# zhoupc/CNMF_E

Hardware: AMD Instinct MI355X
Metric: cnmfe_iters_per_sec (higher is better)
Workload: dtype f32; 1 GPU; c3: 512x512x10000 fp32 video, K=500, ring_radius=15, 1x1 patches of distribute_data.m (1 resident blocks per GPU), spatial=hals, deconv_flag=false, bg_ssub=1; lanes_per_rank=1, parallelism=patches round-robin over 1 rank(s)

## Files before the change

### cnmf_e_amd/csrc/api.hip

```cpp
#include "common.hpp"
#include <mutex>
#include <hip/hip_fp16.h>
#include <math.h>
#include <dlfcn.h>

namespace cnmfe {
thread_local char g_err[1024] = "";

template <class S> __device__ inline float to_f32(S v) { return (float)v; }
template <> __device__ inline float to_f32<__half>(__half v) { return __half2float(v); }

template <class S>
__global__ void k_convert(const S *__restrict__ src, float *__restrict__ dst, int64_t n) {
    int64_t i = (int64_t)blockIdx.x * blockDim.x + threadIdx.x;
    int64_t stride = (int64_t)gridDim.x * blockDim.x;
    for (; i < n; i += stride) dst[i] = to_f32<S>(src[i]);
}

__global__ void k_ymean(const float *__restrict__ Y, int64_t d_b, int64_t T, double *__restrict__ ym, float *__restrict__ ymf) {
    int64_t q = (int64_t)blockIdx.x * blockDim.x + threadIdx.x;
    if (q >= d_b) return;
    double s0 = 0, s1 = 0, s2 = 0, s3 = 0;
    int64_t t = 0;
    for (; t + 3 < T; t += 4) {
        s0 += Y[(t + 0) * d_b + q]; s1 += Y[(t + 1) * d_b + q];
        s2 += Y[(t + 2) * d_b + q]; s3 += Y[(t + 3) * d_b + q];
    }
    for (; t < T; ++t) s0 += Y[t * d_b + q];
    double m = ((s0 + s1) + (s2 + s3)) / (double)T;
    ym[q] = m; ymf[q] = (float)m;
}

__global__ void k_center4(const float *__restrict__ Y, const float *__restrict__ ymf, int64_t d_b, int64_t T, float4 *__restrict__ out) {
    const int64_t q = (int64_t)blockIdx.x * blockDim.x + threadIdx.x;
    if (q >= d_b) return;
    const int64_t c = blockIdx.y;
    const float m = ymf[q];
    const int64_t t = 4 * c;
    float4 v;
    v.x = Y[t * d_b + q] - m;
    v.y = t + 1 < T ? Y[(t + 1) * d_b + q] - m : 0.f;
    v.z = t + 2 < T ? Y[(t + 2) * d_b + q] - m : 0.f;
    v.w = t + 3 < T ? Y[(t + 3) * d_b + q] - m : 0.f;
    out[c * d_b + q] = v;
}

__global__ void k_scratch_warm(int *out, int n) {
    volatile int a[144];
    for (int i = 0; i < 144; ++i) a[i] = i * n;
    int s = 0;
    for (int i = 0; i < n; ++i) s += a[(i * 7 + n) % 144];
    if (out) *out = s;
}

__global__ void k_ring_init(float *__restrict__ W, int64_t d, int nr, int p, const int *__restrict__ dr, const int *__restrict__ dc,
                            int r0, int c0, int d1, int d2) {
    int64_t m = (int64_t)blockIdx.x * blockDim.x + threadIdx.x;
    if (m >= d) return;
    int r = r0 + (int)(m % nr), c = c0 + (int)(m / nr);
    int cnt = 0;
    for (int i = 0; i < p; ++i) { int rr = r + dr[i], cc = c + dc[i]; cnt += (rr >= 1 && rr <= d1 && cc >= 1 && cc <= d2); }
    float v = cnt ? 1.0f / (float)cnt : 0.0f;
    for (int i = 0; i < p; ++i) { int rr = r + dr[i], cc = c + dc[i];
        W[(int64_t)i * d + m] = (rr >= 1 && rr <= d1 && cc >= 1 && cc <= d2) ? v : 0.0f; }
}

__global__ void k_transpose_in(const float *__restrict__ src, float *__restrict__ dst, int K, int64_t T, int64_t ldc) {
    __shared__ float tile[32][33];
    int64_t t0 = (int64_t)blockIdx.x * 32; int k0 = blockIdx.y * 32;
    for (int j = threadIdx.y; j < 32; j += blockDim.y) {
        int64_t t = t0 + j; int k = k0 + threadIdx.x;
        tile[j][threadIdx.x] = (t < T && k < K) ? src[t * K + k] : 0.f;
    }
    __syncthreads();
    for (int j = threadIdx.y; j < 32; j += blockDim.y) {
        int k = k0 + j; int64_t t = t0 + threadIdx.x;
        if (k < K && t < T) dst[(int64_t)k * ldc + t] = tile[threadIdx.x][j];
    }
}
__global__ void k_transpose_out(const float *__restrict__ src, int64_t ldc, float *__restrict__ dst, int K, int64_t T) {
    __shared__ float tile[32][33];
    int64_t t0 = (int64_t)blockIdx.x * 32; int k0 = blockIdx.y * 32;
    for (int j = threadIdx.y; j < 32; j += blockDim.y) {
        int k = k0 + j; int64_t t = t0 + threadIdx.x;
        tile[j][threadIdx.x] = (k < K && t < T) ? src[(int64_t)k * ldc + t] : 0.f;
    }
    __syncthreads();
    for (int j = threadIdx.y; j < 32; j += blockDim.y) {
        int64_t t = t0 + j; int k = k0 + threadIdx.x;
        if (t < T && k < K) dst[t * K + k] = tile[threadIdx.x][j];
    }
}

__global__ void __launch_bounds__(256) k_gather_rows(const float4 *__restrict__ src, int64_t ldc4, const int *__restrict__ idx, float4 *__restrict__ dst) {
    const float4 *s = src + (int64_t)idx[blockIdx.x] * ldc4;
    float4 *d = dst + (int64_t)blockIdx.x * ldc4;
    for (int64_t c = threadIdx.x; c < ldc4; c += 256) d[c] = s[c];
}

int upload_traces(cnmfe_ctx *ctx, DevBuf &dst, const float *C, int32_t K, int64_t T, int order, int64_t *ldc_out) {
    int64_t ldc = (T + 3) & ~int64_t(3);
    *ldc_out = ldc;
    RET(dst.ensure(std::max<int64_t>(1, (int64_t)K * ldc) * sizeof(float)));
    if (K == 0) return 0;
    if (order == CNMFE_BOUND) {
        if (!ctx->bound_valid || ctx->bound_K != K || ctx->bound_T != T)
            return fail(CNMFE_ESTATE, "no bound trace matrix of %d x %lld (cnmfe_traces_bind)", K, (long long)T);
        CK(hipMemcpyAsync(dst.p, ctx->bound.p, (size_t)K * ldc * sizeof(float), hipMemcpyDeviceToDevice, ctx->st()));
        return 0;
    }
    if (!C) return fail(CNMFE_EINVAL, "null trace matrix");
    if (order == CNMFE_BOUND_ROWS) {
        if (!ctx->bound_valid || ctx->bound_T != T) return fail(CNMFE_ESTATE, "no bound trace matrix with %lld frames (cnmfe_traces_bind)", (long long)T);
        const int32_t *rows = reinterpret_cast<const int32_t *>(C);
        for (int32_t k = 0; k < K; ++k)
            if (rows[k] < 0 || rows[k] >= ctx->bound_K) return fail(CNMFE_EINVAL, "row %d of the bound trace matrix (%d rows) does not exist", rows[k], ctx->bound_K);
        DevBuf &dIdx = ctx->tmp[15];
        RET(to_dev(ctx, dIdx, rows, (size_t)K));
        LAUNCH(ctx, "gather_rows", k_gather_rows, dim3((unsigned)K), dim3(256), 0, ctx->bound.as<float4>(), ldc >> 2, dIdx.as<int>(), dst.as<float4>());
        return 0;
    }
    CK(hipMemsetAsync(dst.p, 0, (size_t)K * ldc * sizeof(float), ctx->st()));
    if (order == CNMFE_ROWMAJOR) {
        CK(hipMemcpy2DAsync(dst.p, ldc * sizeof(float), C, T * sizeof(float), T * sizeof(float), K, hipMemcpyDefault, ctx->st()));
    } else {
        RET(ctx->stage.ensure((size_t)K * T * sizeof(float)));
        CK(hipMemcpyAsync(ctx->stage.p, C, (size_t)K * T * sizeof(float), hipMemcpyHostToDevice, ctx->st()));
        dim3 g((unsigned)((T + 31) / 32), (unsigned)((K + 31) / 32)), b(32, 8);
        LAUNCH(ctx, "transpose_in", k_transpose_in, g, b, 0, ctx->stage.as<float>(), dst.as<float>(), K, T, ldc);
    }
    CK(hipStreamSynchronize(ctx->st()));
    return 0;
}

int download_traces(cnmfe_ctx *ctx, const float *dC, int64_t ldc, float *C, int32_t K, int64_t T, int order) {
    if (K == 0 || !C) return 0;
    if (order == CNMFE_BOUND || order == CNMFE_BOUND_ROWS) order = ctx->bound_order;
    if (order == CNMFE_ROWMAJOR) {
        CK(hipMemcpy2DAsync(C, T * sizeof(float), dC, ldc * sizeof(float), T * sizeof(float), K, hipMemcpyDeviceToHost, ctx->st()));
    } else {
        RET(ctx->stage.ensure((size_t)K * T * sizeof(float)));
        dim3 g((unsigned)((T + 31) / 32), (unsigned)((K + 31) / 32)), b(32, 8);
        LAUNCH(ctx, "transpose_out", k_transpose_out, g, b, 0, dC, ldc, ctx->stage.as<float>(), K, T);
        CK(hipMemcpyAsync(C, ctx->stage.p, (size_t)K * T * sizeof(float), hipMemcpyDeviceToHost, ctx->st()));
    }
    CK(hipStreamSynchronize(ctx->st()));
    return 0;
}

__global__ void __launch_bounds__(256) k_pin_copy(PinSegs s) {
    const int g = blockIdx.y;
    const uint4 *__restrict__ src = s.src[g]; uint4 *__restrict__ dst = s.dst[g];
    const unsigned n16 = s.n16[g];
    for (unsigned i = blockIdx.x * 256u + threadIdx.x; i < n16; i += gridDim.x * 256u) dst[i] = src[i];
}
static std::mutex g_pin_mu;
static std::vector<cnmfe_ctx *> g_pin_live;
void pin_register(cnmfe_ctx *ctx, bool live) {
    std::lock_guard<std::mutex> lk(g_pin_mu);
    auto it = std::find(g_pin_live.begin(), g_pin_live.end(), ctx);
    if (live && it == g_pin_live.end()) g_pin_live.push_back(ctx);
    if (!live && it != g_pin_live.end()) g_pin_live.erase(it);
}
static void flush_locked(cnmfe_ctx *ctx) {
    if (!ctx->npseg) return;
    PinSegs &pseg = ctx->pseg;
    unsigned mx = 0;
    for (int i = 0; i < ctx->npseg; ++i) mx = std::max(mx, pseg.n16[i]);
    for (int i = ctx->npseg; i < PIN_NSEG; ++i) { pseg.src[i] = nullptr; pseg.dst[i] = nullptr; pseg.n16[i] = 0; }
    const unsigned nb = std::min<unsigned>((mx + 255) / 256, 256);
    const int n = ctx->npseg; ctx->npseg = 0;
    hipLaunchKernelGGL(k_pin_copy, dim3(nb, (unsigned)n), dim3(256), 0, ctx->stream_, pseg);
}
void pin_flush_range(const void *p, size_t bytes) {
    std::lock_guard<std::mutex> lk(g_pin_mu);
    const char *lo = (const char *)p, *hi = lo + bytes;
    int cur = -1;
    for (cnmfe_ctx *c : g_pin_live) {
        bool hit = false;
        for (int i = 0; i < c->npseg && !hit; ++i) { const char *d_ = (const char *)c->pseg.dst[i]; hit = d_ >= lo && d_ < hi; }
        if (!hit) continue;
        if (cur < 0) (void)hipGetDevice(&cur);
        if (c->device != cur) (void)hipSetDevice(c->device);
        flush_locked(c);
        if (c->device != cur) (void)hipSetDevice(cur);
    }
}
void pin_flush_all() {
    std::lock_guard<std::mutex> lk(g_pin_mu);
    int cur = -1;
    for (cnmfe_ctx *c : g_pin_live) {
        if (!c->npseg) continue;
        if (cur < 0) (void)hipGetDevice(&cur);
        if (c->device != cur) (void)hipSetDevice(c->device);
        flush_locked(c);
        if (c->device != cur) (void)hipSetDevice(cur);
    }
}
int pinned_to_dev(cnmfe_ctx *ctx, void *dst, const void *src_pinned, size_t bytes) {
    if (bytes > (size_t(8) << 20)) { CK(hipMemcpyAsync(dst, src_pinned, bytes, hipMemcpyHostToDevice, ctx->st())); return 0; }
    std::lock_guard<std::mutex> lk(g_pin_mu);
    if (ctx->npseg == PIN_NSEG) flush_locked(ctx);
    const int i = ctx->npseg++;
    ctx->pseg.src[i] = (const uint4 *)src_pinned; ctx->pseg.dst[i] = (uint4 *)dst; ctx->pseg.n16[i] = (unsigned)((bytes + 15) / 16);
    return 0;
}
}
int cnmfe_ctx::copy_batch_mark() {
    hipEvent_t e;
    if (!copy_ev_pool.empty()) { e = copy_ev_pool.back(); copy_ev_pool.pop_back(); }
    else CK(hipEventCreateWithFlags(&e, hipEventDisableTiming));
    CK(hipEventRecord(e, copy_stream));
    copy_gens.push_back({++copy_gen, e});
    return 0;
}
void cnmfe_ctx::flush_copies() {
    std::lock_guard<std::mutex> lk(cnmfe::g_pin_mu);
    cnmfe::flush_locked(this);
}
namespace cnmfe {

bool bound_rows_of(const cnmfe_ctx *ctx, const float *C, int c_order, int32_t K, std::vector<int32_t> &rows) {
    rows.clear();
    if (!ctx->bound_valid || K <= 0) return false;
    if (c_order == CNMFE_BOUND) {
        if (K != ctx->bound_K) return false;
        rows.resize((size_t)K);
        for (int32_t k = 0; k < K; ++k) rows[k] = k;
        return true;
    }
    if (c_order == CNMFE_BOUND_ROWS && C) {
        const int32_t *r = reinterpret_cast<const int32_t *>(C);
        for (int32_t k = 0; k < K; ++k) if (r[k] < 0 || r[k] >= ctx->bound_K) return false;
        rows.assign(r, r + K);
        return true;
    }
    return false;
}

int ensure_ymean(cnmfe_ctx *ctx, Patch *P) {
    if (P->ymean_valid) return 0;
    if (P->frames_uploaded < P->T) return fail(CNMFE_ESTATE, "block has %lld of %lld frames uploaded", (long long)P->frames_uploaded, (long long)P->T);
    RET(P->ymean_d.ensure(P->d_b * sizeof(double)));
    RET(P->ymean_f.ensure(P->d_b * sizeof(float)));
    LAUNCH(ctx, "ymean", k_ymean, dim3((unsigned)((P->d_b + 255) / 256)), dim3(256), 0,
           P->Y.as<float>(), P->d_b, P->T, P->ymean_d.as<double>(), P->ymean_f.as<float>());
    P->Tc = (P->T + 3) / 4;
    RET(P->Yc4.ensure((size_t)P->Tc * P->d_b * sizeof(float4)));
    LAUNCH(ctx, "center4", k_center4, dim3((unsigned)((P->d_b + 255) / 256), (unsigned)P->Tc), dim3(256), 0,
           P->Y.as<float>(), P->ymean_f.as<float>(), P->d_b, P->T, P->Yc4.as<float4>());
    CK(hipStreamSynchronize(ctx->st()));
    (void)hipFree(P->Y.p); P->Y.p = nullptr; P->Y.cap = 0;
    P->ymean_valid = true;
    return 0;
}

__global__ void k_ring_pmax(const float *__restrict__ W, int64_t d, int p, int *__restrict__ pmax) {
    int64_t m = (int64_t)blockIdx.x * blockDim.x + threadIdx.x;
    int c = 0;
    if (m < d) {
        int i = 0;
        for (; i + 16 <= p; i += 16) {
            float w[16];
#pragma unroll
            for (int u = 0; u < 16; ++u) w[u] = W[(int64_t)(i + u) * d + m];
#pragma unroll
            for (int u = 0; u < 16; ++u) c += w[u] > 0.f;
        }
        for (; i < p; ++i) c += W[(int64_t)i * d + m] > 0.f;
    }
    for (int o = 32; o > 0; o >>= 1) { int v = __shfl_xor(c, o); c = v > c ? v : c; }
    if ((threadIdx.x & 63) == 0) atomicMax(pmax, c);
}
static bool first_run_of_row(const Patch *P, const float *row0) {
    std::vector<float> u;
    const int r = P->prect[0], c = P->prect[2];
    int nvalid = 0;
    for (int i = 0; i < P->p; ++i) {
        const int rr = r + P->dr[i], cc = c + P->dc[i];
        if (rr < 1 || rr > P->d1 || cc < 1 || cc > P->d2) continue;
        ++nvalid; u.push_back(row0[i]);
    }
    if (nvalid < P->d_b) u.push_back(0.f);
    std::sort(u.begin(), u.end());
    u.erase(std::unique(u.begin(), u.end()), u.end());
    return u.size() == 2;
}
int ring_stats_enqueue(cnmfe_ctx *ctx, Patch *P) {
    const size_t bytes = 64 + (size_t)P->p * sizeof(float);
    if (!P->stat_host) CK(hipHostMalloc(&P->stat_host, bytes, hipHostMallocDefault));
    if (!P->stat_ev) CK(hipEventCreateWithFlags(&P->stat_ev, hipEventDisableTiming));
    RET(P->stat_dev.ensure(64));
    CK(hipMemsetAsync(P->stat_dev.p, 0, 64, ctx->st()));
    LAUNCH(ctx, "ring_pmax", k_ring_pmax, dim3((unsigned)((P->d + 255) / 256)), dim3(256), 0, P->W.as<float>(), P->d, P->p, P->stat_dev.as<int>());
    CK(hipMemcpyAsync(P->stat_host, P->stat_dev.p, sizeof(int), hipMemcpyDeviceToHost, ctx->st()));
    CK(hipMemcpy2DAsync((char *)P->stat_host + 64, sizeof(float), P->W.p, P->d * sizeof(float), sizeof(float), P->p, hipMemcpyDeviceToHost, ctx->st()));
    CK(hipEventRecord(P->stat_ev, ctx->st()));
    P->stat_valid = true;
    return 0;
}
int ring_stats_get(cnmfe_ctx *ctx, Patch *P, int *pmax, bool *first) {
    if (!P->stat_valid) RET(ring_stats_enqueue(ctx, P));
    CK(hipEventSynchronize(P->stat_ev));
    if (pmax) *pmax = *reinterpret_cast<const int *>(P->stat_host);
    if (first) *first = first_run_of_row(P, reinterpret_cast<const float *>((const char *)P->stat_host + 64));
    return 0;
}

int ring_first_run(cnmfe_ctx *ctx, Patch *P, bool *first) { return ring_stats_get(ctx, P, nullptr, first); }
int ctx_errflag(cnmfe_ctx *ctx, int **dflag) {
    if (!ctx->errflag.p) {
        RET(ctx->errflag.ensure(sizeof(int)));
        CK(hipMemsetAsync(ctx->errflag.p, 0, sizeof(int), ctx->st()));
    }
    *dflag = ctx->errflag.as<int>();
    return 0;
}
static int errflag_raise(cnmfe_ctx *ctx, int h, bool taken = false) {
    if (!taken) CK(hipMemsetAsync(ctx->errflag.p, 0, sizeof(int), ctx->st()));
    for (auto &kv : ctx->patches) { Patch *q = kv.second; q->ysig_valid = false; q->ysig_virtual = false; q->pend = false; q->res_ac = false; q->res_kind = 0; q->pt_valid = false; }
    ctx->bgs_patch = -1;
    if (h & 8) return fail(CNMFE_EHIP, "temporal update: the device's aa = diag(A'A) disagrees with the host-side test of a column (flag %d)", h);
    if (h & 2) return fail(CNMFE_EUNSUPPORTED, "a pixel's ring touches more than 256 footprints of A_prev (flag %d)", h);
    if (h & 4) return fail(CNMFE_EUNSUPPORTED, "bg_ssub > 1: a pixel's interpolation window meets more than 64 footprints of A_prev (flag %d)", h);
    return fail(CNMFE_ESTATE, "a kernel met an inconsistent table (flag %d): the ring regression needed a block pair the covariance table does not hold", h);
}
int ctx_check_errflag(cnmfe_ctx *ctx) {
    if (!ctx->errflag.p) { CK(hipStreamSynchronize(ctx->st())); return 0; }
    int h = 0;
    CK(hipMemcpyAsync(&h, ctx->errflag.p, sizeof(int), hipMemcpyDeviceToHost, ctx->st()));
    CK(hipStreamSynchronize(ctx->st()));
    if (!h) return 0;
    return errflag_raise(ctx, h);
}
__global__ void k_flag_take(int *__restrict__ flag, int *__restrict__ out) { *out = atomicExch(flag, 0); }
__global__ void __launch_bounds__(256) k_fetch_take(const uint4 *__restrict__ src, uint4 *__restrict__ dst, unsigned n16, int *__restrict__ flag, int *__restrict__ flag_out) {
    for (unsigned i = blockIdx.x * 256u + threadIdx.x; i < n16; i += gridDim.x * 256u) dst[i] = src[i];
    if (flag && blockIdx.x == 0 && threadIdx.x == 0) *flag_out = atomicExch(flag, 0);
}

__global__ void __launch_bounds__(256) k_stitch_add(const float *__restrict__ craw, int64_t ldc, const float *__restrict__ aa, const int *__restrict__ ind,
                                                    float *__restrict__ acc, int64_t ld, int64_t T) {
    const int j = blockIdx.y;
    const float w = aa[j];
    float *row = acc + (int64_t)ind[j] * ld;
    const int64_t t = (int64_t)blockIdx.x * 256 + threadIdx.x;
    if (t < T) row[t] += w * craw[(int64_t)j * ldc + t];
    if (t == 0) row[ld - 4] += w;
}
__global__ void __launch_bounds__(256) k_stitch_finish(const float *__restrict__ acc, int64_t ld, int64_t T, int subtract_min, float *__restrict__ out, int64_t ldc) {
    const int k = blockIdx.x;
    const float *row = acc + (int64_t)k * ld;
    float w = row[ld - 4];
    if (w == 0.f) w = 1.f;
    float mn = INFINITY;
    for (int64_t t = threadIdx.x; t < T; t += 256) mn = fminf(mn, row[t] / w);
    __shared__ float red[256];
    red[threadIdx.x] = mn; __syncthreads();
    for (int o = 128; o > 0; o >>= 1) { if ((int)threadIdx.x < o) red[threadIdx.x] = fminf(red[threadIdx.x], red[threadIdx.x + o]); __syncthreads(); }
    const float sub = subtract_min ? red[0] : 0.f;
    for (int64_t t = threadIdx.x; t < ldc; t += 256) out[(int64_t)k * ldc + t] = t < T ? row[t] / w - sub : 0.f;
}

struct Rccl {
    void *h = nullptr;
    int (*CommInitAll)(void **, int, const int *) = nullptr;
    int (*AllReduce)(const void *, void *, size_t, int, int, void *, hipStream_t) = nullptr;
    int (*GroupStart)() = nullptr; int (*GroupEnd)() = nullptr; int (*CommDestroy)(void *) = nullptr;
    const char *(*GetErrorString)(int) = nullptr;
    int load() {
        if (h) return 0;
        for (const char *n : {"librccl.so.1", "librccl.so", "/opt/rocm/lib/librccl.so.1"}) { h = dlopen(n, RTLD_NOW | RTLD_GLOBAL); if (h) break; }
        if (!h) return fail(CNMFE_EUNSUPPORTED, "cnmfe_stitch_temporal over several GPUs needs RCCL (librccl.so not found: %s)", dlerror());
        CommInitAll = (decltype(CommInitAll))dlsym(h, "ncclCommInitAll"); AllReduce = (decltype(AllReduce))dlsym(h, "ncclAllReduce");
        GroupStart = (decltype(GroupStart))dlsym(h, "ncclGroupStart"); GroupEnd = (decltype(GroupEnd))dlsym(h, "ncclGroupEnd");
        CommDestroy = (decltype(CommDestroy))dlsym(h, "ncclCommDestroy"); GetErrorString = (decltype(GetErrorString))dlsym(h, "ncclGetErrorString");
        if (!CommInitAll || !AllReduce || !GroupStart || !GroupEnd || !CommDestroy) { h = nullptr; return fail(CNMFE_EUNSUPPORTED, "librccl.so lacks the ncclCommInitAll / ncclAllReduce / ncclGroup* symbols"); }
        return 0;
    }
};
static Rccl g_rccl;
static int stitch_finish_one(cnmfe_ctx *ctx, int subtract_min, float *C_raw_out, int c_order, bool async_copy = false) {
    if (!ctx->stitch_open) return fail(CNMFE_ESTATE, "cnmfe_stitch_begin has not been called");
    const int32_t K = ctx->stitch_K; const int64_t T = ctx->stitch_T, ldc = (T + 3) & ~int64_t(3);
    CK(hipSetDevice(ctx->device));
    GlobalScope gs_(ctx); if (gs_.rc) return gs_.rc;
    RET(ctx->bound.ensure((size_t)std::max<int64_t>(1, (int64_t)K * ldc) * sizeof(float)));
    if (ctx->copy_pending) { CK(hipStreamWaitEvent(ctx->st(), ctx->ev_copy_done, 0)); ctx->copy_pending = false; }
    if (K > 0) LAUNCH(ctx, "stitch_finish", k_stitch_finish, dim3((unsigned)K), dim3(256), 0, ctx->stitch.as<float>(), ctx->stitch_ld, T, subtract_min, ctx->bound.as<float>(), ldc);
    ctx->bound_K = K; ctx->bound_T = T; ctx->bound_order = (c_order == CNMFE_COLMAJOR) ? CNMFE_COLMAJOR : CNMFE_ROWMAJOR; ctx->bound_valid = K > 0;
    ++ctx->bound_gen;
    ctx->stitch_open = false;
    if (C_raw_out && async_copy && K > 0) {
        if (!ctx->copy_stream) {
            CK(hipStreamCreateWithFlags(&ctx->copy_stream, hipStreamNonBlocking));
            CK(hipEventCreateWithFlags(&ctx->ev_bound_ready, hipEventDisableTiming));
            CK(hipEventCreateWithFlags(&ctx->ev_copy_done, hipEventDisableTiming));
        }
        CK(hipEventRecord(ctx->ev_bound_ready, ctx->st()));
        CK(hipStreamWaitEvent(ctx->copy_stream, ctx->ev_bound_ready, 0));
        CK(hipMemcpy2DAsync(C_raw_out, T * sizeof(float), ctx->bound.p, ldc * sizeof(float), T * sizeof(float), K, hipMemcpyDeviceToHost, ctx->copy_stream));
        CK(hipEventRecord(ctx->ev_copy_done, ctx->copy_stream));
        ctx->copy_pending = true;
        RET(ctx->copy_batch_mark());
        return 0;
    }
    if (C_raw_out) RET(download_traces(ctx, ctx->bound.as<float>(), ldc, C_raw_out, K, T, c_order == CNMFE_COLMAJOR ? CNMFE_COLMAJOR : CNMFE_ROWMAJOR));
    return 0;
}

static void ring_offsets(int radius, int k, std::vector<int32_t> &dr, std::vector<int32_t> &dc) {
    dr.clear(); dc.clear();
    for (int c = -radius; c <= radius; ++c)
        for (int r = -radius; r <= radius; ++r) {
            int d2 = c * c + r * r;
            if (d2 >= radius * radius && d2 < (radius + 1) * (radius + 1)) { dr.push_back(r); dc.push_back(c); }
        }
    int n = (int)dr.size();
    if (k <= 0 || k > n) return;
    std::vector<int> ids(n);
    for (int i = 0; i < n; ++i) ids[i] = i;
    std::vector<double> ang(n);
    for (int i = 0; i < n; ++i) ang[i] = atan2((double)dr[i], (double)dc[i]);
    std::stable_sort(ids.begin(), ids.end(), [&](int a, int b) { return ang[a] < ang[b]; });
    std::vector<std::pair<int, int>> sel;
    for (int j = 0; j < k; ++j) {
        double x = (k == 1) ? 1.0 : 1.0 + (double)(n - 1) * j / (double)(k - 1);
        int idx = (int)floor(x + 0.5) - 1;
        sel.push_back({dc[ids[idx]], dr[ids[idx]]});
    }
    std::sort(sel.begin(), sel.end());
    sel.erase(std::unique(sel.begin(), sel.end()), sel.end());
    dr.clear(); dc.clear();
    for (auto &s : sel) { dc.push_back(s.first); dr.push_back(s.second); }
}
}

using namespace cnmfe;

cnmfe_ctx::~cnmfe_ctx() {
    if (rccl_comm && g_rccl.CommDestroy) { (void)hipSetDevice(device); g_rccl.CommDestroy(rccl_comm); rccl_comm = nullptr; }
    for (auto &kv : patches) delete kv.second;
    prof.drain();
    if (copy_stream) { (void)hipStreamSynchronize(copy_stream); (void)hipStreamDestroy(copy_stream); }
    if (ev_bound_ready) (void)hipEventDestroy(ev_bound_ready);
    if (ev_copy_done) (void)hipEventDestroy(ev_copy_done);
    for (auto &g : copy_gens) (void)hipEventDestroy(g.second);
    for (auto e : copy_ev_pool) (void)hipEventDestroy(e);
    cnmfe::pin_register(this, false);
    for (auto *j : tjobs) delete j;
    for (auto e : tickets) (void)hipEventDestroy(e);
    if (ticket_flags) (void)hipHostFree(ticket_flags);
    if (stream_) (void)hipStreamDestroy(stream_);
    for (auto *L : lanes) delete L;
    if (ev_fork) (void)hipEventDestroy(ev_fork);
}

void cnmfe_ctx::swap_lane(cnmfe_lane &L) {
    std::swap(stream_, L.stream_); std::swap(pseg, L.pseg); std::swap(npseg, L.npseg); pin.swap(L.pin); std::swap(spatial_nnz, L.spatial_nnz);
    for (int i = 0; i < 32; ++i) vp[i].swap(L.vp[i]);
    std::swap(last_ldc, L.last_ldc);
    ysig_low.swap(L.ysig_low); up_tmp.swap(L.up_tmp); bgs_r.swap(L.bgs_r); bgs_b.swap(L.bgs_b); bgs_upr.swap(L.bgs_upr); bgs_upc.swap(L.bgs_upc);
    std::swap(bgs_patch, L.bgs_patch); std::swap(bgs_d1s, L.bgs_d1s); std::swap(bgs_dF, L.bgs_dF);
    bf.swap(L.bf); dig_smax.swap(L.dig_smax); dig_rspart.swap(L.dig_rspart); dig_scale.swap(L.dig_scale); tdig.swap(L.tdig); tscale.swap(L.tscale); gk.swap(L.gk);
    win_items.swap(L.win_items); bf2.swap(L.bf2); outl_cnt.swap(L.outl_cnt); outl_sel.swap(L.outl_sel); cov.swap(L.cov); rowsum.swap(L.rowsum);
    for (int i = 0; i < 16; ++i) tmp[i].swap(L.tmp[i]);
    for (int i = 0; i < 7; ++i) inc[i].swap(L.inc[i]);
    for (int i = 0; i < 4; ++i) stg[i].swap(L.stg[i]);
    wcodes.swap(L.wcodes); solve_fill.swap(L.solve_fill); stage.swap(L.stage);
    for (int i = 0; i < 24; ++i) scr[i].swap(L.scr[i]);
    dscr.swap(L.dscr);
}
int cnmfe_ctx::activate(int lane) {
    if (lanes.empty() || lane == cur_lane) {
        if (!lanes.empty() && lane != 0 && lanes[lane]->fork_seen != fork_gen) {
            CK(hipStreamWaitEvent(stream_, ev_fork, 0)); lanes[lane]->fork_seen = fork_gen;
        }
        if (!lanes.empty() && lane != 0) lanes[lane]->dirty = true;
        return 0;
    }
    if (lane < 0 || lane >= (int)lanes.size()) return fail(CNMFE_ESTATE, "lane %d of %d", lane, (int)lanes.size());
    if (npseg) flush_copies();
    swap_lane(*lanes[cur_lane]);
    swap_lane(*lanes[lane]);
    cur_lane = lane;
    if (lane != 0) {
        if (lanes[lane]->fork_seen != fork_gen) { CK(hipStreamWaitEvent(stream_, ev_fork, 0)); lanes[lane]->fork_seen = fork_gen; }
        lanes[lane]->dirty = true;
    }
    return 0;
}
int cnmfe_ctx::join_lanes() {
    if (lanes.empty()) return 0;
    for (int l = 1; l < (int)lanes.size(); ++l) {
        if (!lanes[l]->dirty) continue;
        RET(activate(l));
        CK(hipEventRecord(lanes[l]->ev, st()));
    }
    RET(activate(0));
    for (int l = 1; l < (int)lanes.size(); ++l)
        if (lanes[l]->dirty) { CK(hipStreamWaitEvent(st(), lanes[l]->ev, 0)); lanes[l]->dirty = false; }
    return 0;
}
int cnmfe_ctx::fork_mark() {
    if (lanes.empty()) return 0;
    RET(activate(0));
    CK(hipEventRecord(ev_fork, st()));
    ++fork_gen;
    return 0;
}
static int lanes_set(cnmfe_ctx *ctx, int64_t n) {
    if (n < 1 || n > 4) return fail(CNMFE_EINVAL, "option lanes = %lld: 1 .. 4", (long long)n);
    if (!ctx->patches.empty() && (int)std::max<size_t>(1, ctx->lanes.size()) != n) return fail(CNMFE_ESTATE, "option lanes is set before the first patch is created");
    if (n == 1 || (int)ctx->lanes.size() == n) return 0;
    CK(hipSetDevice(ctx->device));
    for (int l = 0; l < n; ++l) {
        cnmfe_lane *L = new cnmfe_lane();
        ctx->lanes.push_back(L);
        CK(hipEventCreateWithFlags(&L->ev, hipEventDisableTiming));
        if (l == 0) continue;
        CK(hipStreamCreate(&L->stream_));
        hipLaunchKernelGGL(k_scratch_warm, dim3(1), dim3(64), 0, L->stream_, (int *)nullptr, 3);
        CK(hipStreamSynchronize(L->stream_));
        if (L->pin.init(size_t(64) << 20) != 0) return fail(CNMFE_EHIP, "pinned staging arena (64 MB) of lane %d could not be allocated", l);
    }
    CK(hipEventCreateWithFlags(&ctx->ev_fork, hipEventDisableTiming));
    CK(hipEventRecord(ctx->ev_fork, ctx->st()));
    return 0;
}

extern "C" {

const char *cnmfe_last_error(void) { return g_err; }
const char *cnmfe_version(void) { return "cnmfe-mi355x 0.1 (gfx950)"; }

cnmfe_ctx *cnmfe_create(int device) {
    int n = 0;
    hipError_t e = hipGetDeviceCount(&n);
    if (e != hipSuccess || n <= 0) { fail(CNMFE_EHIP, "no HIP device visible (%s)", hipGetErrorString(e)); return nullptr; }
    if (device < 0 || device >= n) { fail(CNMFE_EINVAL, "device %d out of range (0..%d)", device, n - 1); return nullptr; }
    if (hipSetDevice(device) != hipSuccess) { fail(CNMFE_EHIP, "hipSetDevice(%d) failed", device); return nullptr; }
    cnmfe_ctx *ctx = new cnmfe_ctx();
    ctx->device = device;
    if (hipStreamCreate(&ctx->stream_) != hipSuccess) { fail(CNMFE_EHIP, "hipStreamCreate failed"); delete ctx; return nullptr; }
    if (hipStreamCreateWithFlags(&ctx->copy_stream, hipStreamNonBlocking) != hipSuccess || hipEventCreateWithFlags(&ctx->ev_bound_ready, hipEventDisableTiming) != hipSuccess ||
        hipEventCreateWithFlags(&ctx->ev_copy_done, hipEventDisableTiming) != hipSuccess) { fail(CNMFE_EHIP, "copy stream / events could not be created"); delete ctx; return nullptr; }
    pin_register(ctx, true);
    if (ctx->pin.init(size_t(64) << 20) != 0) { fail(CNMFE_EHIP, "pinned staging arena (64 MB) could not be allocated"); delete ctx; return nullptr; }
    hipLaunchKernelGGL(k_scratch_warm, dim3(1), dim3(64), 0, ctx->stream_, (int *)nullptr, 3);
    hipLaunchKernelGGL(k_scratch_warm, dim3(1), dim3(64), 0, ctx->copy_stream, (int *)nullptr, 3);
    (void)hipStreamSynchronize(ctx->stream_); (void)hipStreamSynchronize(ctx->copy_stream); (void)hipGetLastError();
    (void)tu_warm_resid(); (void)tu_warm_bg(); (void)tu_warm_factor(); (void)tu_warm_deconv(); (void)tu_warm_ssub(); (void)tu_warm_vproj();
    if (const char *env = getenv("CNMFE_OPTS")) {
        std::string s(env), applied, ignored;
        size_t pos = 0;
        while (pos < s.size()) {
            size_t end = s.find(',', pos); if (end == std::string::npos) end = s.size();
            const std::string kv = s.substr(pos, end - pos); pos = end + 1;
            const size_t eq = kv.find('=');
            if (eq == std::string::npos || eq == 0) continue;
            const int rc_ = cnmfe_set_option(ctx, kv.substr(0, eq).c_str(), strtoll(kv.c_str() + eq + 1, nullptr, 10));
            (rc_ == 0 ? applied : ignored) += (rc_ == 0 ? (applied.empty() ? "" : ",") : (ignored.empty() ? "" : ",")) + kv;
        }
        static bool said = false;
        if (!said) { said = true; fprintf(stderr, "[cnmfe] CNMFE_OPTS applied to every context: %s%s%s\n", applied.empty() ? "(none)" : applied.c_str(), ignored.empty() ? "" : "; not known to this build, ignored: ", ignored.c_str()); }
    }
    return ctx;
}

void cnmfe_destroy(cnmfe_ctx *ctx) {
    if (!ctx) return;
    (void)hipSetDevice(ctx->device);
    (void)ctx->join_lanes();
    (void)hipStreamSynchronize(ctx->st());
    delete ctx;
}

int cnmfe_synchronize(cnmfe_ctx *ctx) {
    if (!ctx) return fail(CNMFE_EINVAL, "null context");
    RET(ctx->join_lanes());
    CK(hipStreamSynchronize(ctx->st()));
    if (ctx->copy_stream) CK(hipStreamSynchronize(ctx->copy_stream));
    return ctx_check_errflag(ctx);
}

int cnmfe_set_option(cnmfe_ctx *ctx, const char *name, int64_t value) {
    if (!ctx || !name) return fail(CNMFE_EINVAL, "null argument");
    static const char *known[] = {"r1_variant", "r1_delta", "r1_lazy", "r1_defer", "r1_virtual", "gram_incremental", "prealloc", "solve_packed", "sweep_dag", "win_i8_planes", "solve_staged", "solve_inv", "solve_inv_terms", "gram_i8", "win_i8", "proj_tiled", "proj_i8", "proj_i8_planes", "ssub_virtual", "temporal_early",
                                  "solve_probe", "r1_probe", "deconv_trace", "host_trace", "debug", nullptr};
    if (!strcmp(name, "lanes")) { RET(lanes_set(ctx, value)); ctx->opts[name] = value; return 0; }
    for (int i = 0; known[i]; ++i) if (!strcmp(known[i], name)) { ctx->opts[name] = value; if (!strcmp(name, "host_trace")) ctx->trace_level = (int)value; return 0; }
    return fail(CNMFE_EINVAL, "unknown option '%s'", name);
}

int cnmfe_get_option(cnmfe_ctx *ctx, const char *name, int64_t *value) {
    if (!ctx || !name || !value) return fail(CNMFE_EINVAL, "null argument");
    const struct { const char *n; int64_t v; } counters[] = {{"temporal_early_hits", ctx->early_hits}, {"temporal_early_drops", ctx->early_drops}, {"temporal_early_declined", ctx->early_declined},
                                                              {"temporal_early_entries", ctx->early_nent}, {"temporal_proj_entries", ctx->last_nent}, {"temporal_nowait", ctx->sweep_nowait},
                                                              {"merge_trace_uploads", ctx->merge_uploads},
                                                              {"bound_K", ctx->bound_valid ? (int64_t)ctx->bound_K : 0}, {"bound_T", ctx->bound_valid ? ctx->bound_T : 0}};
    for (const auto &c : counters) if (!strcmp(c.n, name)) { *value = c.v; return 0; }
    auto it = ctx->opts.find(name);
    if (it == ctx->opts.end()) return fail(CNMFE_EINVAL, "option '%s' is unknown or was never set (its default holds)", name);
    *value = it->second;
    return 0;
}

int cnmfe_patch_create(cnmfe_ctx *ctx, int patch_id, const int32_t pr[4], const int32_t br[4], int32_t d1, int32_t d2, int64_t T) {
    if (!ctx || !pr || !br) return fail(CNMFE_EINVAL, "null argument");
    if (d1 <= 0 || d2 <= 0 || T <= 0) return fail(CNMFE_EINVAL, "bad dims d1=%d d2=%d T=%lld", d1, d2, (long long)T);
    if (!(1 <= br[0] && br[0] <= pr[0] && pr[0] <= pr[1] && pr[1] <= br[1] && br[1] <= d1 &&
          1 <= br[2] && br[2] <= pr[2] && pr[2] <= pr[3] && pr[3] <= br[3] && br[3] <= d2))
        return fail(CNMFE_EINVAL, "patch [%d %d %d %d] must lie inside block [%d %d %d %d] inside the %dx%d FOV",
                    pr[0], pr[1], pr[2], pr[3], br[0], br[1], br[2], br[3], d1, d2);
    CK(hipSetDevice(ctx->device));
    if (ctx->patches.count(patch_id)) { delete ctx->patches[patch_id]; ctx->patches.erase(patch_id); }
    ctx->early.valid = false; ctx->spatial_patch = nullptr;
    Patch *P = new Patch();
    P->lane = ctx->lanes.empty() ? 0 : (ctx->patches_created++ % (int)ctx->lanes.size());
    memcpy(P->prect, pr, sizeof(P->prect)); memcpy(P->brect, br, sizeof(P->brect));
    P->d1 = d1; P->d2 = d2; P->T = T;
    P->nr = pr[1] - pr[0] + 1; P->nc = pr[3] - pr[2] + 1;
    P->nr_b = br[1] - br[0] + 1; P->nc_b = br[3] - br[2] + 1;
    P->roff = pr[0] - br[0]; P->coff = pr[2] - br[2];
    P->d = (int64_t)P->nr * P->nc; P->d_b = (int64_t)P->nr_b * P->nc_b;
    int rc = P->Y.ensure((size_t)P->d_b * T * sizeof(float));
    if (rc) { delete P; return rc; }
    if (hipMemsetAsync(P->Y.p, 0, (size_t)P->d_b * T * sizeof(float), ctx->st()) != hipSuccess) { delete P; return fail(CNMFE_EHIP, "hipMemsetAsync of the upload staging failed"); }
    P->frame_seen.assign((size_t)T, 0);
    P->Tc = (T + 3) / 4;
    ctx->patches[patch_id] = P;
    return 0;
}

int cnmfe_upload_block(cnmfe_ctx *ctx, int patch_id, const void *Y, int dtype, int memspace, int64_t t0, int64_t nt) {
    if (!ctx || !Y) return fail(CNMFE_EINVAL, "null argument");
    Patch *P = get_patch(ctx, patch_id);
    if (!P) return fail(CNMFE_ESTATE, "patch %d not created", patch_id);
    if (t0 < 0 || nt <= 0 || t0 + nt > P->T) return fail(CNMFE_EINVAL, "frames [%lld,%lld) outside [0,%lld)", (long long)t0, (long long)(t0 + nt), (long long)P->T);
    CK(hipSetDevice(ctx->device));
    size_t esz = dtype == CNMFE_F32 ? 4 : dtype == CNMFE_F64 ? 8 : dtype == CNMFE_U16 ? 2 : dtype == CNMFE_U8 ? 1 : dtype == CNMFE_F16 ? 2 : 0;
    if (!esz) return fail(CNMFE_EINVAL, "unknown dtype %d", dtype);
    if (memspace != CNMFE_HOST && memspace != CNMFE_DEVICE) return fail(CNMFE_EINVAL, "unknown memspace %d", memspace);
    if (!P->Y.p) {
        RET(P->Y.ensure((size_t)P->d_b * P->T * sizeof(float)));
        CK(hipMemsetAsync(P->Y.p, 0, (size_t)P->d_b * P->T * sizeof(float), ctx->st()));
        P->frames_uploaded = 0;
        P->frame_seen.assign((size_t)P->T, 0);
    }
    for (int64_t t = t0; t < t0 + nt; ++t)
        if (P->frame_seen[(size_t)t]) return fail(CNMFE_EINVAL, "frame %lld of patch %d was already uploaded (chunks must not overlap; re-create the patch to replace its video)", (long long)t, patch_id);
    float *dst = P->Y.as<float>() + t0 * P->d_b;
    int64_t n = nt * P->d_b;
    if (dtype == CNMFE_F32) {
        CK(hipMemcpyAsync(dst, Y, (size_t)n * 4, memspace == CNMFE_HOST ? hipMemcpyHostToDevice : hipMemcpyDeviceToDevice, ctx->st()));
    } else {
        const int64_t slab = int64_t(1) << 26;
        for (int64_t o = 0; o < n; o += slab) {
            int64_t m = std::min(slab, n - o);
            const void *src = (const char *)Y + (size_t)o * esz;
            if (memspace == CNMFE_HOST) {
                RET(ctx->stage.ensure((size_t)m * esz));
                CK(hipMemcpyAsync(ctx->stage.p, src, (size_t)m * esz, hipMemcpyHostToDevice, ctx->st()));
                src = ctx->stage.p;
            }
            dim3 g((unsigned)std::min<int64_t>((m + 255) / 256, 65535)), b(256);
            switch (dtype) {
                case CNMFE_F64: LAUNCH(ctx, "convert", k_convert<double>, g, b, 0, (const double *)src, dst + o, m); break;
                case CNMFE_U16: LAUNCH(ctx, "convert", k_convert<uint16_t>, g, b, 0, (const uint16_t *)src, dst + o, m); break;
                case CNMFE_U8:  LAUNCH(ctx, "convert", k_convert<uint8_t>, g, b, 0, (const uint8_t *)src, dst + o, m); break;
                default:        LAUNCH(ctx, "convert", k_convert<__half>, g, b, 0, (const __half *)src, dst + o, m); break;
            }
            if (memspace == CNMFE_HOST) CK(hipStreamSynchronize(ctx->st()));
        }
    }
    CK(hipStreamSynchronize(ctx->st()));
    std::fill(P->frame_seen.begin() + t0, P->frame_seen.begin() + t0 + nt, (uint8_t)1);
    P->frames_uploaded += nt;
    P->ymean_valid = false; P->ysig_valid = false; P->base_valid = false; P->base_alt_valid = false; P->drop_systems(); P->sys_alt_valid = false; P->pt_valid = false; P->dig_valid = false; P->digp_valid = false; P->yt4_valid = false;
    return 0;
}

int cnmfe_get_ymean(cnmfe_ctx *ctx, int patch_id, double *out) {
    if (!ctx || !out) return fail(CNMFE_EINVAL, "null argument");
    Patch *P = get_patch(ctx, patch_id);
    if (!P) return fail(CNMFE_ESTATE, "patch %d not created", patch_id);
    CK(hipSetDevice(ctx->device));
    RET(ensure_ymean(ctx, P));
    CK(hipMemcpyAsync(out, P->ymean_d.p, P->d_b * sizeof(double), hipMemcpyDeviceToHost, ctx->st()));
    CK(hipStreamSynchronize(ctx->st()));
    return 0;
}

int cnmfe_ring_init(cnmfe_ctx *ctx, int patch_id, int32_t radius, int32_t num_neighbors) {
    if (!ctx) return fail(CNMFE_EINVAL, "null context");
    Patch *P = get_patch(ctx, patch_id);
    if (!P) return fail(CNMFE_ESTATE, "patch %d not created", patch_id);
    if (radius < 1 || radius > 64) return fail(CNMFE_EINVAL, "ring radius %d out of range", radius);
    CK(hipSetDevice(ctx->device));
    std::vector<int32_t> ndr, ndc;
    ring_offsets(radius, num_neighbors, ndr, ndc);
    const int32_t np_ = (int32_t)ndr.size();
    if (np_ < 1) return fail(CNMFE_EINVAL, "ring of radius %d has no neighbours", radius);
    if (np_ > PMAX_RING) return fail(CNMFE_EUNSUPPORTED, "ring with %d neighbours exceeds the supported %d", np_, PMAX_RING);
    if (radius > 24) return fail(CNMFE_EUNSUPPORTED, "ring radius %d: the block-pair covariance table of the ring regression covers radii <= 24", radius);
    int h = radius;
    if ((P->prect[0] - P->brect[0] < std::min(h, P->prect[0] - 1)) || (P->brect[1] - P->prect[1] < std::min(h, P->d1 - P->prect[1])) ||
        (P->prect[2] - P->brect[2] < std::min(h, P->prect[2] - 1)) || (P->brect[3] - P->prect[3] < std::min(h, P->d2 - P->prect[3])))
        return fail(CNMFE_EINVAL, "block halo is narrower than the ring radius %d", radius);
    P->ring_ready = false;
    P->dr.swap(ndr); P->dc.swap(ndc); P->p = np_; P->radius = radius;
    RET(to_dev(ctx, P->ring_dr, P->dr.data(), P->dr.size()));
    RET(to_dev(ctx, P->ring_dc, P->dc.data(), P->dc.size()));
    RET(P->W.ensure((size_t)P->p * P->d * sizeof(float)));
    RET(P->b0.ensure(P->d * sizeof(double)));
    CK(hipMemsetAsync(P->b0.p, 0, P->d * sizeof(double), ctx->st()));
    LAUNCH(ctx, "ring_init", k_ring_init, dim3((unsigned)((P->d + 255) / 256)), dim3(256), 0,
           P->W.as<float>(), P->d, P->nr, P->p, P->ring_dr.as<int>(), P->ring_dc.as<int>(), P->prect[0], P->prect[2], P->d1, P->d2);
    CK(hipStreamSynchronize(ctx->st()));
    P->stat_valid = false;
    if (P->stat_host) { (void)hipHostFree(P->stat_host); P->stat_host = nullptr; }
    P->ring_ready = true; P->ysig_valid = false; P->base_valid = false; P->base_alt_valid = false; P->drop_systems(); P->sys_alt_valid = false; P->pt_valid = false;
    return 0;
}

static int64_t ring_count_nnz(const Patch *P) {
    int64_t nnz = 0;
    for (int i = 0; i < P->p; ++i) {
        int64_t rlo = std::max<int64_t>(P->prect[0], 1 - P->dr[i]), rhi = std::min<int64_t>(P->prect[1], P->d1 - P->dr[i]);
        int64_t clo = std::max<int64_t>(P->prect[2], 1 - P->dc[i]), chi = std::min<int64_t>(P->prect[3], P->d2 - P->dc[i]);
        if (rhi >= rlo && chi >= clo) nnz += (rhi - rlo + 1) * (chi - clo + 1);
    }
    return nnz;
}

int cnmfe_ring_nnz(cnmfe_ctx *ctx, int patch_id, int64_t *nnz, int32_t *p) {
    if (!ctx) return fail(CNMFE_EINVAL, "null context");
    Patch *P = get_patch(ctx, patch_id);
    if (!P || !P->ring_ready) return fail(CNMFE_ESTATE, "ring of patch %d not initialised", patch_id);
    if (nnz) *nnz = ring_count_nnz(P);
    if (p) *p = P->p;
    return 0;
}

int cnmfe_ring_get_csr(cnmfe_ctx *ctx, int patch_id, int64_t *rowptr, int32_t *col, float *val) {
    if (!ctx || !rowptr || !col || !val) return fail(CNMFE_EINVAL, "null argument");
    Patch *P = get_patch(ctx, patch_id);
    if (!P || !P->ring_ready) return fail(CNMFE_ESTATE, "ring of patch %d not initialised", patch_id);
    CK(hipSetDevice(ctx->device));
    std::vector<float> W((size_t)P->p * P->d);
    CK(hipMemcpyAsync(W.data(), P->W.p, W.size() * sizeof(float), hipMemcpyDeviceToHost, ctx->st()));
    CK(hipStreamSynchronize(ctx->st()));
    int64_t e = 0;
    for (int64_t m = 0; m < P->d; ++m) {
        rowptr[m] = e;
        int r = P->prect[0] + (int)(m % P->nr), c = P->prect[2] + (int)(m / P->nr);
        for (int i = 0; i < P->p; ++i) {
            int rr = r + P->dr[i], cc = c + P->dc[i];
            if (rr < 1 || rr > P->d1 || cc < 1 || cc > P->d2) continue;
            col[e] = (int32_t)((int64_t)(cc - P->brect[2]) * P->nr_b + (rr - P->brect[0]));
            val[e] = W[(size_t)i * P->d + m];
            ++e;
        }
    }
    rowptr[P->d] = e;
    return 0;
}

int cnmfe_ring_set_values(cnmfe_ctx *ctx, int patch_id, const float *val) {
    if (!ctx || !val) return fail(CNMFE_EINVAL, "null argument");
    Patch *P = get_patch(ctx, patch_id);
    if (!P || !P->ring_ready) return fail(CNMFE_ESTATE, "ring of patch %d not initialised", patch_id);
    CK(hipSetDevice(ctx->device));
    std::vector<float> W((size_t)P->p * P->d, 0.f);
    int64_t e = 0;
    for (int64_t m = 0; m < P->d; ++m) {
        int r = P->prect[0] + (int)(m % P->nr), c = P->prect[2] + (int)(m / P->nr);
        for (int i = 0; i < P->p; ++i) {
            int rr = r + P->dr[i], cc = c + P->dc[i];
            if (rr < 1 || rr > P->d1 || cc < 1 || cc > P->d2) continue;
            W[(size_t)i * P->d + m] = val[e++];
        }
    }
    CK(hipMemcpyAsync(P->W.p, W.data(), W.size() * sizeof(float), hipMemcpyHostToDevice, ctx->st()));
    CK(hipStreamSynchronize(ctx->st()));
    P->stat_valid = false;
    P->ysig_valid = false;
    return 0;
}

int cnmfe_ring_first_run(cnmfe_ctx *ctx, int patch_id, int *first_run) {
    if (!ctx || !first_run) return fail(CNMFE_EINVAL, "null argument");
    Patch *P = get_patch(ctx, patch_id);
    if (!P || !P->ring_ready) return fail(CNMFE_ESTATE, "ring of patch %d not initialised", patch_id);
    CK(hipSetDevice(ctx->device));
    bool f = false;
    RET(ring_first_run(ctx, P, &f));
    *first_run = f ? 1 : 0;
    return 0;
}

int cnmfe_b0_get(cnmfe_ctx *ctx, int patch_id, float *b0) {
    if (!ctx || !b0) return fail(CNMFE_EINVAL, "null argument");
    Patch *P = get_patch(ctx, patch_id);
    if (!P || !P->ring_ready) return fail(CNMFE_ESTATE, "ring of patch %d not initialised", patch_id);
    CK(hipSetDevice(ctx->device));
    std::vector<double> tmp(P->d);
    CK(hipMemcpyAsync(tmp.data(), P->b0.p, P->d * sizeof(double), hipMemcpyDeviceToHost, ctx->st()));
    CK(hipStreamSynchronize(ctx->st()));
    for (int64_t i = 0; i < P->d; ++i) b0[i] = (float)tmp[i];
    return 0;
}

int cnmfe_b0_set(cnmfe_ctx *ctx, int patch_id, const float *b0) {
    if (!ctx || !b0) return fail(CNMFE_EINVAL, "null argument");
    Patch *P = get_patch(ctx, patch_id);
    if (!P || !P->ring_ready) return fail(CNMFE_ESTATE, "ring of patch %d not initialised", patch_id);
    CK(hipSetDevice(ctx->device));
    std::vector<double> tmp(P->d);
    for (int64_t i = 0; i < P->d; ++i) tmp[i] = (double)b0[i];
    CK(hipMemcpyAsync(P->b0.p, tmp.data(), P->d * sizeof(double), hipMemcpyHostToDevice, ctx->st()));
    CK(hipStreamSynchronize(ctx->st()));
    P->ysig_valid = false;
    return 0;
}

static int check_csc(const char *what, int32_t K, int64_t nrow, const int64_t *colptr, const int32_t *rowidx) {
    if (K < 0) return fail(CNMFE_EINVAL, "%s: K=%d", what, K);
    if (K == 0) return 0;
    if (!colptr) return fail(CNMFE_EINVAL, "%s: null colptr", what);
    if (colptr[0] != 0) return fail(CNMFE_EINVAL, "%s: colptr[0] != 0", what);
    for (int32_t k = 0; k < K; ++k) if (colptr[k + 1] < colptr[k]) return fail(CNMFE_EINVAL, "%s: colptr not monotone at %d", what, k);
    int64_t nnz = colptr[K];
    if (nnz && !rowidx) return fail(CNMFE_EINVAL, "%s: null rowidx", what);
    for (int32_t k = 0; k < K; ++k)
        for (int64_t e = colptr[k]; e < colptr[k + 1]; ++e) {
            if (rowidx[e] < 0 || rowidx[e] >= nrow) return fail(CNMFE_EINVAL, "%s: row index %d out of [0,%lld)", what, rowidx[e], (long long)nrow);
            if (e > colptr[k] && rowidx[e] <= rowidx[e - 1]) return fail(CNMFE_EINVAL, "%s: rows of column %d not strictly ascending", what, k);
        }
    return 0;
}
extern "C++" { namespace cnmfe { int check_csc_pub(const char *what, int32_t ncol, int64_t nrow, const int64_t *colptr, const int32_t *rowidx) { return check_csc(what, ncol, nrow, colptr, rowidx); } } }

int cnmfe_ring_solve_stats(cnmfe_ctx *ctx, int patch_id, int64_t out[4]) {
    if (!ctx || !out) return fail(CNMFE_EINVAL, "null argument");
    Patch *P = get_patch(ctx, patch_id);
    if (!P) return fail(CNMFE_EINVAL, "no patch %d", patch_id);
    out[0] = out[1] = out[2] = out[3] = -1;
    if (!P->kinv_valid || !P->kinv_list.p) return 0;
    CK(hipSetDevice(ctx->device));
    int h[4];
    CK(hipMemcpyAsync(h, P->kinv_list.as<int>() + 2 * P->d, sizeof(h), hipMemcpyDeviceToHost, ctx->st()));
    CK(hipStreamSynchronize(ctx->st()));
    for (int i = 0; i < 4; ++i) out[i] = h[i];
    return 0;
}

int cnmfe_fit_ring_model(cnmfe_ctx *ctx, int patch_id, int32_t K, const int64_t *A_colptr, const int32_t *A_rowidx,
                         const float *A_val, const float *C, int c_order, double thresh_outlier, int with_projection,
                         float *b0_out, int64_t info[4]) {
    if (!ctx) return fail(CNMFE_EINVAL, "null context");
    Patch *P = get_patch(ctx, patch_id);
    if (!P || !P->ring_ready) return fail(CNMFE_ESTATE, "ring of patch %d not initialised", patch_id);
    RET(check_csc("A", K, P->d_b, A_colptr, A_rowidx));
    if (K > 0 && ((!A_val && A_colptr[K] > 0) || (!C && c_order != CNMFE_BOUND))) return fail(CNMFE_EINVAL, "null A_val / C");
    CK(hipSetDevice(ctx->device));
    RET(ensure_ymean(ctx, P));
    int64_t dummy[4];
    int rc = bg_fit_ring(ctx, P, K, A_colptr, A_rowidx, A_val, C, c_order, with_projection, b0_out, info ? info : dummy, 0, thresh_outlier);
    P->ysig_valid = false;
    return rc;
}

int cnmfe_fit_reserve(cnmfe_ctx *ctx, int patch_id) {
    if (!ctx) return fail(CNMFE_EINVAL, "null context");
    Patch *P = get_patch(ctx, patch_id);
    if (!P || !P->ring_ready) return fail(CNMFE_ESTATE, "ring of patch %d not initialised", patch_id);
    CK(hipSetDevice(ctx->device));
    if (ctx->opt("prealloc", 1) == 0) return 0;
    return bg_reserve(ctx, P);
}

int cnmfe_set_noise(cnmfe_ctx *ctx, int patch_id, const float *sn_block) {
    if (!ctx) return fail(CNMFE_EINVAL, "null context");
    Patch *P = get_patch(ctx, patch_id);
    if (!P) return fail(CNMFE_ESTATE, "patch %d not created", patch_id);
    if (!sn_block) return fail(CNMFE_EINVAL, "null sn_block");
    CK(hipSetDevice(ctx->device));
    RET(to_dev(ctx, P->sn_b, sn_block, (size_t)P->d_b));
    CK(hipStreamSynchronize(ctx->st()));
    P->sn_ready = true;
// ... 842 lines not shown
```

### cnmf_e_amd/csrc/bg.hip

```cpp
#include "common.hpp"
#include "ring_solve_core.hpp"
#include "win_proj.hpp"
#include <type_traits>

namespace cnmfe {
static inline bool win_planes3(cnmfe_ctx *ctx, int64_t T16) {
    const int64_t o = ctx->opt("win_i8_planes", 0);
    return o == 3 || (o != 4 && T16 * 16 >= 2048);
}


typedef float float4_t __attribute__((ext_vector_type(4)));

__global__ void __launch_bounds__(256) k_build_bf(const float4 *__restrict__ Y4, int64_t Tc, BgGeom g,
                                                  const int *__restrict__ arow, const int *__restrict__ acol, const float *__restrict__ aval,
                                                  const float *__restrict__ Cc, int64_t ldc, float *__restrict__ bf, int tchunk, double *__restrict__ rs) {
    const int blk = blockIdx.x;
    const int bi = blk % g.nbr, bj = blk / g.nbr;
    const int lp = threadIdx.x;
    const int lr = ((lp >> 4) & 3) * 4 + (lp & 3), lc = (lp >> 6) * 4 + ((lp >> 2) & 3);
    const int rb = bi * BLK + lr, cb = bj * BLK + lc;
    const bool in = rb < g.nr_b && cb < g.nc_b;
    const int64_t q = in ? (int64_t)cb * g.nr_b + rb : 0;
    int e0 = 0, e1 = 0;
// ... 107 lines not shown
            const int cur = (base >> 1) & 1;
            if (base + 2 < NS) ldb(cur ^ 1, base + 2);
            asm volatile("" ::: "memory");
            const bool on0 = true, on1 = (base + 1 < NS - 1) || (base + 1 == NS - 1 && last);
            const bool only0_last = (base == NS - 1);
            const bool do0 = only0_last ? last : on0;
#pragma unroll
            for (int kq = 0; kq < 4; ++kq) {
#pragma unroll
                for (int u = 0; u < 2; ++u) {
                    if (base + u >= NS) continue;
                    if (u == 0 ? !do0 : !on1) continue;
                    const float av = kq == 0 ? fa[cur][u].x : kq == 1 ? fa[cur][u].y : kq == 2 ? fa[cur][u].z : fa[cur][u].w;
                    const float bv = kq == 0 ? fb[cur][u].x : kq == 1 ? fb[cur][u].y : kq == 2 ? fb[cur][u].z : fb[cur][u].w;
                    acc[base + u] = __builtin_amdgcn_mfma_f64_16x16x4f64((double)av, (double)bv, acc[base + u], 0, 0, 0);
                }
            }
        }
        asm volatile("" ::: "memory");
    }
    asm volatile("s_waitcnt vmcnt(0)" ::: "memory");
    const int fl = w.lane & 15;
#pragma unroll
    for (int sl = 0; sl < NS; ++sl)
        if (sl < NS - 1 || last) {
#pragma unroll
            for (int r = 0; r < 4; ++r) {
                const int rr = (w.lane >> 4) + 4 * r;
                w.out[(int64_t)(ti[sl] * 16 + rr) * BLKPX + tj[sl] * 16 + fl] = acc[sl][r];
            }
        }
}

__global__ void __launch_bounds__(256, 2) k_gram4(const float *__restrict__ bf, int64_t Tpad, const int4 *__restrict__ pairs,
                                                  const int *__restrict__ work, int nwork, const int *__restrict__ tl_cnt,
                                                  const int *__restrict__ tl, int probe, double *__restrict__ cov) {
    extern __shared__ __attribute__((aligned(16))) float smem[];
    const int nwg = gridDim.x;
    int bid = blockIdx.x;
    if (nwg % 8 == 0) bid = (blockIdx.x % 8) * (nwg / 8) + blockIdx.x / 8;
    if (bid >= nwork) return;
    const int wk = work[bid];
    const int pair = wk >> 2, quad = wk & 3;
    const int ih = quad & 1, jh = quad >> 1;
    const int4 pr = pairs[pair];
    const int tid = threadIdx.x, lane = tid & 63;
    const int wave = __builtin_amdgcn_readfirstlane(tid >> 6);
    const int lidx = pr.z * 4 + quad;
    const int cnt = __builtin_amdgcn_readfirstlane(tl_cnt[lidx]);
    G4Wave w;
    w.gA = bf + ((int64_t)pr.x * Tpad) * BLKPX + ih * 512;
    w.gB = bf + ((int64_t)pr.y * Tpad) * BLKPX + jh * 512;
    w.vo0 = (unsigned)((((wave >> 1) * BLKPX + (wave & 1) * 64 + lane) * 4) * 4);
    w.vo1 = w.vo0 + 2u * BLKPX * 4u * 4u;
    w.dA0 = (unsigned)(uintptr_t)(__attribute__((address_space(3))) float *)smem + (unsigned)wave * 1024u;
    w.lbase = (lane >> 4) * 512 + (lane & 15) * 4;
    w.nst = (int)(Tpad / GK); w.probe = probe; w.lane = lane;
    w.ns = cnt > wave ? (cnt - wave + 3) >> 2 : 0;
    w.out = cov + (int64_t)pair * BLKPX * BLKPX + (int64_t)(ih * 128) * BLKPX + jh * 128;
    const int *tlw = tl + lidx * 64 + wave;
    switch ((cnt + 3) >> 2) {
#define G4_CASE(N) case N: gram4_run<N>(w, smem, tlw); break;
        G4_CASE(1) G4_CASE(2) G4_CASE(3) G4_CASE(4) G4_CASE(5) G4_CASE(6) G4_CASE(7) G4_CASE(8)
        G4_CASE(9) G4_CASE(10) G4_CASE(11) G4_CASE(12) G4_CASE(13) G4_CASE(14) G4_CASE(15) G4_CASE(16)
#undef G4_CASE
        default: break;
    }
}

__global__ void __launch_bounds__(256) k_trace_subsum(const float *__restrict__ Cc, int64_t ldc, int64_t Tp, int kstride, double *__restrict__ csum) {
    const float *row = Cc + (int64_t)blockIdx.x * ldc;
    __shared__ double red[256];
    double s = 0;
    for (int64_t tp = threadIdx.x; tp < Tp; tp += 256) s += (double)row[tp * kstride];
    red[threadIdx.x] = s; __syncthreads();
    for (int o = 128; o > 0; o >>= 1) { if ((int)threadIdx.x < o) red[threadIdx.x] += red[threadIdx.x + o]; __syncthreads(); }
    if (threadIdx.x == 0) csum[blockIdx.x] = red[0];
}

template <int NT>
__device__ __forceinline__ void win_body(const float4 *__restrict__ Y4, const BgGeom &g, const float *__restrict__ Cc, int64_t ldc, int blk, int l0, int nl,
                                         const int *__restrict__ lst_k, int64_t c0, int64_t c1, double *__restrict__ Ut, double *__restrict__ Gb) {
    const int bi = blk % g.nbr, bj = blk / g.nbr;
    const int tid = threadIdx.x, lane = tid & 63, wave = tid >> 6, fi = lane & 15, kq = lane >> 4;
    const float *Ys = reinterpret_cast<const float *>(Y4);
    const float *ya[4]; const float *tb[NT];
#pragma unroll
    for (int a = 0; a < 4; ++a) {
        const int lp = (wave * 4 + a) * 16 + fi;
        const int lr = ((lp >> 4) & 3) * 4 + (lp & 3), lc = (lp >> 6) * 4 + ((lp >> 2) & 3);
        const int rb = bi * BLK + lr, cb = bj * BLK + lc;
        ya[a] = (rb < g.nr_b && cb < g.nc_b) ? Ys + ((int64_t)cb * g.nr_b + rb) * 4 : nullptr;
    }
#pragma unroll
    for (int b = 0; b < NT; ++b) { const int sl = b * 16 + fi; tb[b] = sl < nl ? Cc + (int64_t)lst_k[l0 + sl] * ldc : nullptr; }
    double4_t acc[4][NT], accg[NT];
#pragma unroll
    for (int b = 0; b < NT; ++b) {
        accg[b] = (double4_t){0.0, 0.0, 0.0, 0.0};
#pragma unroll
        for (int a = 0; a < 4; ++a) acc[a][b] = (double4_t){0.0, 0.0, 0.0, 0.0};
    }
    struct Frag { float y[4]; float t[NT]; };
    auto load = [&](int64_t c) {
        Frag f;
        const int64_t tp = 4 * c + kq, t = tp * g.kstride;
        const bool on = c < c1 && tp < g.Tp;
        const int64_t yo = ((t >> 2) * g.d_b) * 4 + (t & 3);
#pragma unroll
        for (int a = 0; a < 4; ++a) f.y[a] = (on && ya[a]) ? ya[a][yo] : 0.f;
#pragma unroll
        for (int b = 0; b < NT; ++b) f.t[b] = (on && tb[b]) ? tb[b][t] : 0.f;
        return f;
    };
    const bool gw = wave < NT;
    auto mm = [&](const Frag &f) {
        double bv[NT];
#pragma unroll
        for (int b = 0; b < NT; ++b) bv[b] = (double)f.t[b];
#pragma unroll
        for (int a = 0; a < 4; ++a) {
            const double av = (double)f.y[a];
#pragma unroll
            for (int b = 0; b < NT; ++b) acc[a][b] = __builtin_amdgcn_mfma_f64_16x16x4f64(av, bv[b], acc[a][b], 0, 0, 0);
        }
        if (gw) {
            double gv = bv[0];
#pragma unroll
            for (int b = 1; b < NT; ++b) gv = wave == b ? bv[b] : gv;
#pragma unroll
            for (int b = 0; b < NT; ++b) accg[b] = __builtin_amdgcn_mfma_f64_16x16x4f64(gv, bv[b], accg[b], 0, 0, 0);
        }
    };
    Frag f[WIN_AHEAD];
#pragma unroll
    for (int d = 0; d < WIN_AHEAD; ++d) f[d] = load(c0 + d);
    for (int64_t c = c0; c < c1; c += WIN_AHEAD) {
#pragma unroll
        for (int d = 0; d < WIN_AHEAD; ++d) {
            const Frag nx = load(c + WIN_AHEAD + d);
            mm(f[d]);
            f[d] = nx;
        }
    }
#pragma unroll
    for (int b = 0; b < NT; ++b) {
        const int slot = b * 16 + fi;
#pragma unroll
        for (int a = 0; a < 4; ++a)
            if (slot < nl)
#pragma unroll
                for (int r = 0; r < 4; ++r) Ut[(int64_t)(l0 + slot) * BLKPX + (wave * 4 + a) * 16 + kq + 4 * r] = acc[a][b][r];
        if (gw)
#pragma unroll
            for (int r = 0; r < 4; ++r) Gb[(int64_t)blk * WIN_NLB * WIN_NLB + (wave * 16 + kq + 4 * r) * WIN_NLB + slot] = accg[b][r];
    }
}

__global__ void __launch_bounds__(256) k_win_proj(const float4 *__restrict__ Y4, BgGeom g, const float *__restrict__ Cc, int64_t ldc, const int *__restrict__ lst_ptr,
                                                  const int *__restrict__ lst_k, const int *__restrict__ blk_list, int nseg, double *__restrict__ Ut, int64_t ut_stride,
                                                  double *__restrict__ Gb, int64_t gb_stride) {
    const int blk = blk_list[blockIdx.x / nseg], seg = blockIdx.x % nseg;
    const int l0 = lst_ptr[blk], nl = lst_ptr[blk + 1] - l0;
    double *ut = Ut + seg * ut_stride, *gb = Gb + seg * gb_stride;
    const int64_t nchunk = (g.Tp + 3) >> 2;
    int64_t cseg = ((nchunk + nseg - 1) / nseg + 1) & ~int64_t(1);
    const int64_t c0 = seg * cseg, c1 = c0 + cseg < nchunk ? c0 + cseg : nchunk;
    switch ((nl + 15) >> 4) {
        case 1: win_body<1>(Y4, g, Cc, ldc, blk, l0, nl, lst_k, c0, c1, ut, gb); break;
        case 2: win_body<2>(Y4, g, Cc, ldc, blk, l0, nl, lst_k, c0, c1, ut, gb); break;
        case 3: win_body<3>(Y4, g, Cc, ldc, blk, l0, nl, lst_k, c0, c1, ut, gb); break;
        case 4: win_body<4>(Y4, g, Cc, ldc, blk, l0, nl, lst_k, c0, c1, ut, gb); break;
        default: break;
    }
}

constexpr int WF_S = 4;
__global__ void __launch_bounds__(256) k_win_fix(BgGeom g, int K, const int *__restrict__ arow, const int *__restrict__ acol, const float *__restrict__ aval,
                                                 const int *__restrict__ lst_ptr, const short *__restrict__ slot_of, const int *__restrict__ blk_list, int nseg,
                                                 double *__restrict__ Ut, int64_t ut_stride, const double *__restrict__ Gb, int64_t gb_stride, double *__restrict__ Praw,
                                                 const double *__restrict__ GK, const int *__restrict__ lst_k) {
    __shared__ double G[WIN_NLB * WF_S];
    const int blk = blk_list[blockIdx.x];
    const int l0 = lst_ptr[blk], nl = lst_ptr[blk + 1] - l0;
    const int s0 = (int)blockIdx.y * WF_S;
    if (s0 >= nl) return;
    const int lp = threadIdx.x;
    const int nlp = ((nl + 15) >> 4) << 4;
    {
        const int r = lp / WF_S, c = s0 + lp % WF_S;
        double v = 0.0;
        if (GK) {
            if (r < nl && c < nl) v = GK[(int64_t)lst_k[l0 + r] * K + lst_k[l0 + c]];
        } else if (r < nlp && c < nlp) {
            const double *gp = Gb + (int64_t)blk * WIN_NLB * WIN_NLB + r * WIN_NLB + c;
#pragma unroll 4
            for (int sg = 0; sg < nseg; ++sg) v += gp[sg * gb_stride];
        }
        G[lp] = v;
    }
    __syncthreads();
    const int lr = ((lp >> 4) & 3) * 4 + (lp & 3), lc = (lp >> 6) * 4 + ((lp >> 2) & 3);
    const int rb = (blk % g.nbr) * BLK + lr, cb = (blk / g.nbr) * BLK + lc;
    int e0 = 0, e1 = 0;
    if (rb < g.nr_b && cb < g.nc_b) { const int64_t q = (int64_t)cb * g.nr_b + rb; e0 = arow[q]; e1 = arow[q + 1]; }
    const int s1 = s0 + WF_S < nl ? s0 + WF_S : nl;
    for (int s = s0; s < s1; ++s) {
        double *u = Ut + (int64_t)(l0 + s) * BLKPX + lp;
        double v = u[0];
#pragma unroll 4
        for (int sg = 1; sg < nseg; ++sg) v += u[sg * ut_stride];
        double w = 0.0;
        for (int e = e0; e < e1; ++e) w += (double)aval[e] * G[(int)slot_of[(int64_t)blk * K + acol[e]] * WF_S + (s - s0)];
        u[0] = v - 0.5 * w;
        if (Praw) Praw[(int64_t)(l0 + s) * BLKPX + lp] = v;
    }
}
static_assert(WIN_NLB * WF_S == 256, "k_win_fix: one Gram entry per thread");

__global__ void __launch_bounds__(256) k_cov_correct(const double *__restrict__ base, double *__restrict__ cov, const int4 *__restrict__ pairs,
                                                     const unsigned short *__restrict__ needmask, BgGeom g, int K, const int *__restrict__ arow,
                                                     const int *__restrict__ acol, const float *__restrict__ aval, const int *__restrict__ lst_ptr,
                                                     const short *__restrict__ slot_of, const double *__restrict__ Ut) {
    const int pair = blockIdx.x;
    const int4 pr = pairs[pair];
    const int ba = pr.x, bb = pr.y, rel = pr.z;
    const int half = threadIdx.x >> 7, ty = (threadIdx.x >> 3) & 15, tx = (threadIdx.x & 7) * 2;
    const int la = lst_ptr[ba], lb = lst_ptr[bb];
    auto pix = [&](int blk, int lp, int &e0, int &e1) {
        const int lr = ((lp >> 4) & 3) * 4 + (lp & 3), lc = (lp >> 6) * 4 + ((lp >> 2) & 3);
        const int rb = (blk % g.nbr) * BLK + lr, cb = (blk / g.nbr) * BLK + lc;
        e0 = e1 = 0;
        if (rb < g.nr_b && cb < g.nc_b) { const int64_t q = (int64_t)cb * g.nr_b + rb; e0 = arow[q]; e1 = arow[q + 1]; }
    };
    const double *bp = base + (int64_t)pair * BLKPX * BLKPX;
    double *cp = cov + (int64_t)pair * BLKPX * BLKPX;
    const int pi0 = (int)blockIdx.y * (16 / (int)gridDim.y), pi1 = pi0 + 16 / (int)gridDim.y;
    for (int pi = pi0 + half; pi < pi1; pi += 2) {
        const unsigned mask = needmask[rel * 16 + pi];
        if (!mask) continue;
        const int ilp = pi * 16 + ty;
        int ei0, ei1; pix(ba, ilp, ei0, ei1);
        for (int pj = 0; pj < 16; ++pj) {
            if (!((mask >> pj) & 1u)) continue;
            const int jlp = pj * 16 + tx;
            int ej0, ej1, ek0, ek1; pix(bb, jlp, ej0, ej1); pix(bb, jlp + 1, ek0, ek1);
            const int idx = ilp * BLKPX + jlp;
            double2 v = *reinterpret_cast<const double2 *>(bp + idx);
            for (int e = ej0; e < ej1; ++e) v.x -= (double)aval[e] * Ut[(int64_t)(la + slot_of[(int64_t)ba * K + acol[e]]) * BLKPX + ilp];
            for (int e = ek0; e < ek1; ++e) v.y -= (double)aval[e] * Ut[(int64_t)(la + slot_of[(int64_t)ba * K + acol[e]]) * BLKPX + ilp];
            for (int e = ei0; e < ei1; ++e) {
                const double2 u = *reinterpret_cast<const double2 *>(Ut + (int64_t)(lb + slot_of[(int64_t)bb * K + acol[e]]) * BLKPX + jlp);
                v.x -= (double)aval[e] * u.x; v.y -= (double)aval[e] * u.y;
            }
            *reinterpret_cast<double2 *>(cp + idx) = v;
        }
    }
}

__global__ void __launch_bounds__(256) k_rowsum_correct(const double *__restrict__ base, double *__restrict__ rs, BgGeom g, const int *__restrict__ arow,
                                                        const int *__restrict__ acol, const float *__restrict__ aval, const double *__restrict__ csum) {
    const int blk = blockIdx.x, lp = threadIdx.x;
    const int lr = ((lp >> 4) & 3) * 4 + (lp & 3), lc = (lp >> 6) * 4 + ((lp >> 2) & 3);
    const int rb = (blk % g.nbr) * BLK + lr, cb = (blk / g.nbr) * BLK + lc;
    double v = base[(int64_t)blk * BLKPX + lp];
    if (rb < g.nr_b && cb < g.nc_b) {
        const int64_t q = (int64_t)cb * g.nr_b + rb;
        for (int e = arow[q]; e < arow[q + 1]; ++e) v -= (double)aval[e] * csum[acol[e]];
    }
    rs[(int64_t)blk * BLKPX + lp] = v;
}

struct CovTab {
    const double *cov; const int *pair_of;
    const int *wcodes; int woff;
    int nbr, nbc;
    int maxd, nrel;
};

__global__ void __launch_bounds__(256) k_win_codes(const int *__restrict__ pair_of, int nbr, int nbc, int woff, int maxd, int nrel, int *__restrict__ wcodes) {
    const int br0 = (int)(blockIdx.x % (nbr + 2 * woff)) - woff, bc0 = (int)(blockIdx.x / (nbr + 2 * woff)) - woff;
    const int q = threadIdx.x, a = q >> 4, b = q & 15;
    int ia = br0 + (a & 3), ja = bc0 + (a >> 2), ib = br0 + (b & 3), jb = bc0 + (b >> 2);
    int code = -1;
    if (ia >= 0 && ja >= 0 && ib >= 0 && jb >= 0 && ia < nbr && ib < nbr && ja < nbc && jb < nbc) {
        int dR = ib - ia, dC = jb - ja, sw = 0;
        if (dC < 0 || (dC == 0 && dR < 0)) { sw = 1; ia = ib; ja = jb; dR = -dR; dC = -dC; }
        if (dC <= maxd && dR <= maxd && dR >= -maxd) {
            const int pidx = pair_of[(ja * nbr + ia) * nrel + rel_index(dR, dC, maxd)];
            code = pidx < 0 ? -1 : ((pidx << 2) | (sw << 1) | ((dR == 0 && dC == 0) ? 1 : 0));
        }
    }
    wcodes[(int64_t)blockIdx.x * 256 + q] = code;
}
}
#include "ring_solve.hpp"
#include "ring_solve_packed.hpp"
#include "ring_solve_inv.hpp"
#include "ring_solve_staged.hpp"
#include "gram_i8.hpp"
#include "win_proj_i8.hpp"
namespace cnmfe {

__global__ void k_active(const float *__restrict__ W, BgGeom g, const int *__restrict__ dr, const int *__restrict__ dc,
                         const float *__restrict__ asum, unsigned char *__restrict__ active, int *__restrict__ nactive) {
    int64_t m = (int64_t)blockIdx.x * blockDim.x + threadIdx.x;
    int on = 0;
    if (m < g.d) {
        const int rbm = (int)(m % g.nr) + g.roff, cbm = (int)(m / g.nr) + g.coff;
        float s = 0.f;
        for (int i0 = 0; i0 < g.p; i0 += 8) {
            float w8[8], a8[8];
#pragma unroll
            for (int u = 0; u < 8; ++u) {
                const int i = i0 + u < g.p ? i0 + u : g.p - 1;
                const int rb = rbm + dr[i], cb = cbm + dc[i];
                const bool in = i0 + u < g.p && rb >= 0 && rb < g.nr_b && cb >= 0 && cb < g.nc_b;
                w8[u] = W[(int64_t)i * g.d + m];
                a8[u] = asum[in ? (int64_t)cb * g.nr_b + rb : 0];
                if (!in) w8[u] = 0.f;
            }
#pragma unroll
            for (int u = 0; u < 8; ++u) if (w8[u] != 0.f) s += fabsf(w8[u]) * a8[u];
        }
        on = s > 0.f;
        active[m] = (unsigned char)on;
    }
    unsigned long long b = __ballot(on);
    if ((threadIdx.x & 63) == 0) atomicAdd(nactive, (int)__popcll(b));
}

__global__ void k_b0(const double *__restrict__ ymean, BgGeom g, const int *__restrict__ arow, const int *__restrict__ acol,
                     const float *__restrict__ aval, const double *__restrict__ Cmean, double *__restrict__ b0) {
    int64_t m = (int64_t)blockIdx.x * blockDim.x + threadIdx.x;
    if (m >= g.d) return;
    const int64_t q = (int64_t)((int)(m / g.nr) + g.coff) * g.nr_b + (int)(m % g.nr) + g.roff;
    double v = ymean[q];
    if (arow) for (int e = arow[q]; e < arow[q + 1]; ++e) v -= (double)aval[e] * Cmean[acol[e]];
    b0[m] = v;
}

__device__ __forceinline__ int64_t bf4_index(const BgGeom &g, int rb, int cb, int64_t c) {
    return ((int64_t)((cb >> 4) * g.nbr + (rb >> 4)) * (g.Tpad >> 2) + c) * BLKPX + lp_of(rb & 15, cb & 15);
}
__global__ void __launch_bounds__(256) k_outlier_clip(const float4 *__restrict__ bf, float4 *__restrict__ bf2, BgGeom g, const int *__restrict__ dr,
                                                      const int *__restrict__ dc, const float *__restrict__ W, const float *__restrict__ sn_b,
                                                      double thresh, int *__restrict__ cnt) {
    const int64_t m = (int64_t)blockIdx.x * blockDim.x + threadIdx.x, c = blockIdx.y;
    if (m >= g.d) return;
    const int rbm = (int)(m % g.nr) + g.roff, cbm = (int)(m / g.nr) + g.coff;
    double o0 = 0, o1 = 0, o2 = 0, o3 = 0;
    for (int i = 0; i < g.p; ++i) {
        const float w = W[(int64_t)i * g.d + m];
        if (w == 0.f) continue;
        const float4 v = bf[bf4_index(g, rbm + dr[i], cbm + dc[i], c)];
        o0 += (double)w * v.x; o1 += (double)w * v.y; o2 += (double)w * v.z; o3 += (double)w * v.w;
    }
    const int64_t at = bf4_index(g, rbm, cbm, c);
    float4 y = bf[at];
    const double lim = thresh * (double)sn_b[(int64_t)cbm * g.nr_b + rbm];
    const int64_t t = c * 4;
    if (t < g.T && (double)y.x > o0 + lim) { y.x = (float)o0; atomicAdd(&cnt[t], 1); }
    if (t + 1 < g.T && (double)y.y > o1 + lim) { y.y = (float)o1; atomicAdd(&cnt[t + 1], 1); }
    if (t + 2 < g.T && (double)y.z > o2 + lim) { y.z = (float)o2; atomicAdd(&cnt[t + 2], 1); }
    if (t + 3 < g.T && (double)y.w > o3 + lim) { y.w = (float)o3; atomicAdd(&cnt[t + 3], 1); }
    bf2[at] = y;
}
__global__ void __launch_bounds__(256) k_select_frames(const float *__restrict__ src, int64_t Tpad_src, float *__restrict__ dst, int64_t Tpad_dst,
                                                       const int *__restrict__ sel, int64_t nsel) {
    const int64_t blk = blockIdx.x, lp = threadIdx.x;
    for (int64_t c = blockIdx.y; c < (Tpad_dst >> 2); c += gridDim.y) {
        float v[4];
        for (int i = 0; i < 4; ++i) {
            const int64_t j = c * 4 + i;
            float x = 0.f;
            if (j < nsel) { const int64_t t = sel[j]; x = src[((blk * (Tpad_src >> 2) + (t >> 2)) * BLKPX + lp) * 4 + (t & 3)]; }
            v[i] = x;
        }
        reinterpret_cast<float4 *>(dst)[(blk * (Tpad_dst >> 2) + c) * BLKPX + lp] = make_float4(v[0], v[1], v[2], v[3]);
    }
}
static double matlab_quantile(std::vector<int> x, double q) {
    std::sort(x.begin(), x.end());
    const int64_t n = (int64_t)x.size();
    const double r = q * (double)n + 0.5;
    if (r <= 1.0) return x[0];
    if (r >= (double)n) return x[n - 1];
    const int64_t lo = (int64_t)std::floor(r);
    return x[lo - 1] + (r - (double)lo) * (double)(x[lo] - x[lo - 1]);
}

template <int MAX, class F> static int nt_dispatch(int nt, F &&f) {
#define NT_CASE(N_) case N_: if constexpr (N_ <= MAX) return f(std::integral_constant<int, N_>{}); else return 0;
    switch (nt) { NT_CASE(1) NT_CASE(2) NT_CASE(3) NT_CASE(4) NT_CASE(5) NT_CASE(6) NT_CASE(7) NT_CASE(8) default: return 0; }
#undef NT_CASE
}
#define NT_OF(c) decltype(c)::value

static int solve_launch(cnmfe_ctx *ctx, Patch *P, const CovTab &tab, const BgGeom &g, const double *rowsum, const unsigned char *act, int nt, int probe, const double *fill) {
    int *dErr = nullptr;
    RET(ctx_errflag(ctx, &dErr));
    return nt_dispatch<8>(nt, [&](auto c) -> int {
        LAUNCH(ctx, "bg_ring_solve", (k_ring_solve5<NT_OF(c)>), dim3((unsigned)P->d), dim3(64), 0, tab, g, P->ring_dr.as<int>(), P->ring_dc.as<int>(), rowsum, act, P->W.as<float>(), dErr, probe, (const int *)nullptr, fill);
        return 0; });
}

int fits_leaving(const DevBuf &b, size_t bytes, bool *fits, bool quarter) {
    *fits = true;
    if (b.cap >= bytes) return 0;
    size_t fr = 0, tot = 0; CK(hipMemGetInfo(&fr, &tot));
    *fits = fr >= bytes + std::max((size_t)8 << 30, quarter ? tot / 4 : (size_t)0);
    return 0;
}
static int fit_stride(int64_t T, int pmax) { return (int)std::max<int64_t>(1, T / std::max<int64_t>(1, std::min<int64_t>(T, (int64_t)pmax * 100))); }
static bool gram_i8_ok(cnmfe_ctx *ctx, int64_t Tp) { return ctx->opt("gram_i8", 1) != 0 && Tp <= 24576; }
static bool planes_wanted(cnmfe_ctx *ctx, const Patch *P, int kstride) { return kstride == 1 && !P->derived && ctx->opt("win_i8", 1) != 0; }
static bool win_i8_applies(cnmfe_ctx *ctx, const Patch *P, int kstride) { return P->dig_valid && kstride == 1 && P->T <= 24576 && ctx->opt("win_i8", 1) != 0; }
static bool pack_wanted(cnmfe_ctx *ctx, int nt) { return ctx->opt("solve_packed", 1) != 0 && nt >= 1 && nt <= 8; }
static size_t sys_bytes_of(int64_t d, int nt) { return (size_t)d * ((size_t)(nt * (nt + 1) / 2) * 256 + 16 * nt) * sizeof(double); }

static int trace_digits(cnmfe_ctx *ctx, const char *name, const float *dCc, int64_t ldc, int K, int64_t T, int64_t T16, bool gram) {
    RET(ctx->tdig.ensure((size_t)K * T16 * 4 * sizeof(uint4))); RET(ctx->tscale.ensure((size_t)K * sizeof(double)));
    if (gram) RET(ctx->gk.ensure((size_t)K * K * sizeof(double)));
    LAUNCH(ctx, name, k_trace_dig, dim3(K), dim3(256), 0, dCc, ldc, T, T16, ctx->tdig.as<uint4>(), ctx->tscale.as<double>());
    if (gram) LAUNCH(ctx, "bg_trace_gram", k_trace_gram, dim3((unsigned)(((K + 15) >> 4) * (((K + 15) >> 4) + 1) / 2)), dim3(64 * TG_W), 0, dCc, ldc, T, K, ctx->gk.as<double>());
    return 0;
}
static int win_proj_i8_launch(cnmfe_ctx *ctx, Patch *P, const char *name, const std::vector<int> &lst_ptr, const std::vector<int> &blall, const int *dLp, const int *dLk, int nsg,
                              double *dUt, int64_t ut_stride) {
    static thread_local std::vector<int> items;
    plan::win_i8_items(blall, lst_ptr, items);
    RET(to_dev(ctx, ctx->win_items, items));
    if (items.empty()) return 0;
    const int64_t T16 = P->dig_T16;
#define WPI8_GO(V0_) LAUNCH(ctx, name, k_win_proj_i8<V0_>, dim3((unsigned)(items.size() * nsg)), dim3(512), 0, P->dig.as<uint4>(), T16, P->dig_sc.as<double>(), ctx->tdig.as<uint4>(), \
                            ctx->tscale.as<double>(), dLp, dLk, ctx->win_items.as<int>(), nsg, dUt, ut_stride)
    if (win_planes3(ctx, T16)) WPI8_GO(1); else WPI8_GO(0);
#undef WPI8_GO
    return 0;
}
static int build_digits(cnmfe_ctx *ctx, Patch *P, const BgGeom &g, const DigA &da, double *digs, uint4 *digp, int *nchunk) {
    const int nblk = g.nbr * g.nbc;
    RET(ctx->dig_smax.ensure((size_t)nblk * BLKPX * sizeof(unsigned)));
    CK(hipMemsetAsync(ctx->dig_smax.p, 0, (size_t)nblk * BLKPX * sizeof(unsigned), ctx->st()));
    const int tchunk16 = (int)((std::max<int64_t>(64, (g.Tpad + 15) / 16) + 15) & ~int64_t(15));
    const dim3 gd(nblk, (unsigned)((g.Tpad + tchunk16 - 1) / tchunk16));
    LAUNCH(ctx, "bg_dig_scale", k_dig_scale, gd, dim3(256), 0, P->Yc4.as<float4>(), P->Tc, g, da, tchunk16, ctx->dig_smax.as<unsigned>());
    if (nchunk) { RET(ctx->dig_rspart.ensure((size_t)gd.y * nblk * BLKPX * sizeof(double))); *nchunk = (int)gd.y; }
    LAUNCH(ctx, "bg_build_dig", k_build_dig, gd, dim3(256), 0, P->Yc4.as<float4>(), P->Tc, g, da, ctx->dig_smax.as<unsigned>(), digs, digp, tchunk16,
           nchunk ? ctx->dig_rspart.as<double>() : (double *)nullptr);
    return 0;
}

int bg_reserve(cnmfe_ctx *ctx, Patch *P) {
    if (ctx->opt("gram_incremental", 1) == 0 || P->p <= 0) return 0;
    const plan::Reach reach = plan::ring_reach(P->dr.data(), P->dc.data(), P->p);
    if (!reach.ok) return 0;
    const bool i8 = gram_i8_ok(ctx, P->T);
    const BgGeom g = bg_geom(P, 1, i8);
    const int nblk = g.nbr * g.nbc, nt = (P->p + 15) / 16;
    const size_t tab = (size_t)plan::ring_pairs(P->nr_b, P->nc_b, P->roff, P->coff, P->nr, P->nc, reach.p_radius, reach.maxd, nullptr, nullptr) * BLKPX * BLKPX * sizeof(double);
    RET(P->cov_base.ensure(tab)); RET(P->rowsum_base.ensure((size_t)nblk * BLKPX * sizeof(double))); RET(ctx->cov.ensure(tab));
    RET(ctx->rowsum.ensure((size_t)nblk * BLKPX * sizeof(double))); RET(ctx->bf.ensure((size_t)nblk * g.Tpad * BLKPX * sizeof(float)));
    RET(ctx->inc[6].ensure((size_t)plan::win_segments(nblk) * nblk * WIN_NLB * WIN_NLB * sizeof(double)));
    bool fits = false;
    if (pack_wanted(ctx, nt) && P->sys.cap < sys_bytes_of(P->d, nt)) {
        RET(fits_leaving(P->sys, sys_bytes_of(P->d, nt), &fits));
        if (fits) { P->drop_systems(); RET(P->sys.ensure(sys_bytes_of(P->d, nt))); }
    }
    auto reserve = [&](DevBuf &b, size_t bytes) -> int { RET(fits_leaving(b, bytes, &fits, true)); return fits ? b.ensure(bytes) : 0; };
    if (P->derived) return 0;
    const bool planes = i8 && planes_wanted(ctx, P, fit_stride(P->T, P->p));
    if (planes) { RET(reserve(P->dig, (size_t)nblk * g.Tpad * BLKPX * sizeof(float))); RET(P->dig_sc.ensure((size_t)nblk * BLKPX * sizeof(double))); }
    if (ctx->opt("r1_virtual", 1) != 0) {
        if (planes && ctx->opt("proj_i8", 1) != 0) RET(reserve(P->digp, (size_t)nblk * g.Tpad * BLKPX * sizeof(float)));
        else if (ctx->opt("proj_tiled", 1) != 0) RET(reserve(P->yt4, (size_t)nblk * ((P->Tc + 15) >> 4) * 64 * 64 * sizeof(float4)));
    }
    return 0;
}

struct RingFit {
    cnmfe_ctx *ctx; Patch *P; int32_t K; const int64_t *A_colptr; const int32_t *A_rowidx; const float *A_val; const float *C; int c_order, b0_only; double thresh_outlier;
    HostTrace ht;
    bool outl, has_a, a_empty;
    int64_t T, ldc = 4, nactive = 0;
    HostCSR csr;
    bool first_run = false; int pmax = 0, kstride = 1;
    BgGeom g; plan::Reach reach; int nblk = 0, nt = 0;
    plan::BlockLists L; std::vector<plan::Pair> pairs; std::vector<int> pair_of; plan::Tables tabs; int npairs = 0, nwork = 0;
    bool incr = false, build_base = false, use_i8 = false, keep_pt = false, trace_i8_done = false, proj_queued = false, win_i8 = false, packed = false, stage_ok = false;
    int nsg = 1; int64_t ut_stride = 0, gb_stride = 0;
    uint4 *digp = nullptr; double *digs = nullptr;
    DevBuf &dC, &dCc, &dCm, &dArow, &dAcol, &dAval, &dMisc, &dAsum, &dActive, &dPairs, &dPairOf, &dWork, &dNeed, &dTcnt, &dTl, &dLk, &dBl, &dUt, &dCsum, &dGb, *dLp, *dSlot;
    RingFit(cnmfe_ctx *c, Patch *p_) : ctx(c), P(p_), ht(c, "fit_ring"), dC(c->tmp[0]), dCc(c->tmp[1]), dCm(c->tmp[2]), dArow(c->tmp[3]), dAcol(c->tmp[4]), dAval(c->tmp[5]), dMisc(c->tmp[6]),
        dAsum(c->tmp[7]), dActive(c->tmp[8]), dPairs(c->tmp[9]), dPairOf(c->tmp[10]), dWork(c->tmp[11]), dNeed(c->tmp[7]), dTcnt(c->tmp[12]), dTl(c->tmp[13]), dLk(c->inc[1]),
        dBl(c->inc[3]), dUt(c->inc[4]), dCsum(c->inc[5]), dGb(c->inc[6]), dLp(&c->inc[0]), dSlot(&c->inc[2]) {}
    const int *arow() const { return has_a ? dArow.as<int>() : nullptr; }
    CovTab covtab() const { CovTab t{}; t.cov = ctx->cov.as<double>(); t.pair_of = dPairOf.as<int>(); t.nbr = g.nbr; t.nbc = g.nbc; t.maxd = reach.maxd; t.nrel = reach.nrel; return t; }
};
static thread_local std::vector<int> fit_nbox;

static int fit_traces_up(RingFit &f) {
    cnmfe_ctx *ctx = f.ctx; Patch *P = f.P;
    if (!f.has_a) return 0;
    RET(upload_centered(ctx, f.dC, f.C, f.K, f.T, f.c_order, f.dCc, f.dCm, &f.ldc));
    if (!f.outl && ctx->opt("gram_incremental", 1) != 0 && win_i8_applies(ctx, P, P->base_valid ? P->base_kstride : 1)) {
        RET(trace_digits(ctx, "bg_trace_dig", f.dCc.as<float>(), f.ldc, f.K, f.T, P->dig_T16, true));
        f.trace_i8_done = true;
    }
    return 0;
}
static int fit_upload_csr(RingFit &f) {
    if (!f.has_a) return 0;
    csc_to_csr(f.P->d_b, f.K, f.A_colptr, f.A_rowidx, f.A_val, f.csr);
    RET(to_dev(f.ctx, f.dArow, f.csr.rowptr)); RET(to_dev(f.ctx, f.dAcol, f.csr.col)); RET(to_dev(f.ctx, f.dAval, f.csr.val));
    return 0;
}
static int fit_b0(RingFit &f, const BgGeom &g) {
    LAUNCH(f.ctx, "bg_b0", k_b0, dim3((unsigned)((f.P->d + 255) / 256)), dim3(256), 0, f.P->ymean_d.as<double>(), g, f.arow(), f.dAcol.as<int>(), f.dAval.as<float>(), f.dCm.as<double>(),
           f.P->b0.as<double>());
    return 0;
}
static int fit_geometry(RingFit &f, int with_projection) {
    RET(ring_stats_get(f.ctx, f.P, &f.pmax, &f.first_run));
    RET(f.dMisc.ensure(64));
    f.ht.mark("first_run + pmax");
    f.kstride = with_projection && !f.outl ? fit_stride(f.T, f.pmax) : 1;
    f.g = bg_geom(f.P, f.kstride);
    f.reach = plan::ring_reach(f.P->dr.data(), f.P->dc.data(), f.P->p);
    f.nblk = f.g.nbr * f.g.nbc; f.nt = (f.P->p + 15) / 16;
    if (!f.reach.ok) return fail(CNMFE_EUNSUPPORTED, "fit_ring_model: ring offsets up to %d pixels (the block-pair table covers <= 24)", f.reach.p_radius);
    return 0;
}
static void fit_lists(RingFit &f) {
    cnmfe_ctx *ctx = f.ctx; Patch *P = f.P;
    static thread_local std::vector<int> pair_blk, k_ptr;
    f.incr = !f.outl && ctx->opt("gram_incremental", 1) != 0 && f.K < 32768;
    if (f.incr) {
        plan::footprint_blocks(f.K, f.A_colptr, f.A_rowidx, P->nr_b, f.g.nbr, f.g.nbc, f.reach.maxd, pair_blk, k_ptr, fit_nbox);
        f.incr = plan::block_lists(f.nblk, f.K, pair_blk.data(), k_ptr.data(), f.L);
    }
    if (f.incr && P->base_valid && P->base_kstride != f.kstride) {
        P->cov_base.swap(P->cov_base_alt); P->rowsum_base.swap(P->rowsum_base_alt);
        std::swap(P->base_valid, P->base_alt_valid); std::swap(P->base_kstride, P->base_alt_kstride);
        P->sys.swap(P->sys_alt); std::swap(P->sys_valid, P->sys_alt_valid);
        P->drop_inverses();
    }
    f.build_base = f.incr && !(P->base_valid && P->base_kstride == f.kstride);
    if (f.build_base) P->drop_systems();
    f.ht.mark("footprint block lists");
    f.use_i8 = (f.build_base || !f.incr) && !f.outl && gram_i8_ok(ctx, f.g.Tp);
    geom_frames(f.g, f.g.Tp, f.use_i8);
    f.keep_pt = f.incr && f.has_a && f.kstride == 1 && !P->derived && !(f.b0_only & 2) && ctx->opt("r1_virtual", 1) != 0;
    if (f.keep_pt) { f.dLp = &P->pt_lp; f.dSlot = &P->pt_slot; P->pt_valid = false; }
}
static int fit_queue_projection(RingFit &f) {
    cnmfe_ctx *ctx = f.ctx; Patch *P = f.P; const BgGeom &g = f.g;
    RET(to_dev(ctx, *f.dLp, f.L.lst_ptr)); RET(to_dev(ctx, f.dLk, f.L.lst_k)); RET(to_dev(ctx, f.dBl, f.L.blall)); RET(f.dCsum.ensure((size_t)f.K * sizeof(double)));
    LAUNCH(ctx, "bg_trace_subsum", k_trace_subsum, dim3(f.K), dim3(256), 0, f.dCc.as<float>(), f.ldc, g.Tp, g.kstride, f.dCsum.as<double>());
    const int nb_ = (int)f.L.blall.size(), nbig = (int)f.L.blk_nt[3].size();
    f.nsg = plan::win_segments(nb_);
    f.ut_stride = (int64_t)std::max<size_t>(1, f.L.lst_k.size()) * BLKPX; f.gb_stride = (int64_t)f.nblk * WIN_NLB * WIN_NLB;
    RET(f.dUt.ensure((size_t)f.nsg * f.ut_stride * sizeof(double))); RET(f.dGb.ensure((size_t)f.nsg * f.gb_stride * sizeof(double)));
    const int *dLp = f.dLp->as<int>(), *dLk = f.dLk.as<int>(), *dBl = f.dBl.as<int>();
    if (win_i8_applies(ctx, P, g.kstride)) {
        if (!f.trace_i8_done) RET(trace_digits(ctx, "bg_trace_dig", f.dCc.as<float>(), f.ldc, f.K, f.T, P->dig_T16, true));
        RET(win_proj_i8_launch(ctx, P, "bg_win_proj", f.L.lst_ptr, f.L.blall, dLp, dLk, f.nsg, f.dUt.as<double>(), f.ut_stride));
        f.win_i8 = true;
    } else if (g.kstride == 1 || g.kstride == 2 || g.kstride == 4)
        RET(win_proj4_launch(ctx, "bg_win_proj", P, g, f.dCc.as<float>(), f.ldc, dLp, dLk, dBl, nbig, nb_, f.nsg, f.dUt.as<double>(), f.ut_stride, f.dGb.as<double>(), f.gb_stride));
    else
        LAUNCH(ctx, "bg_win_proj", k_win_proj, dim3((unsigned)(nb_ * f.nsg)), dim3(256), 0, P->Yc4.as<float4>(), g, f.dCc.as<float>(), f.ldc, dLp, dLk, dBl, f.nsg, f.dUt.as<double>(), f.ut_stride,
               f.dGb.as<double>(), f.gb_stride);
    f.proj_queued = true;
    return 0;
}
static int fit_active_b0(RingFit &f) {
    cnmfe_ctx *ctx = f.ctx; Patch *P = f.P;
    RET(f.dActive.ensure(P->d));
    f.nactive = P->d;
    if (f.first_run) { CK(hipMemsetAsync(f.dActive.p, 1, P->d, ctx->st())); } else {
        std::vector<float> asum(P->d_b, 0.f);
        if (f.a_empty || (f.b0_only & 2)) std::fill(asum.begin(), asum.end(), 1.0f);
        else if (f.has_a) for (int64_t q = 0; q < P->d_b; ++q) { double s = 0; for (int64_t e = f.csr.rowptr[q]; e < f.csr.rowptr[q + 1]; ++e) s += f.csr.val[e]; asum[q] = (float)s; }
        RET(to_dev(ctx, f.dAsum, asum));
        CK(hipMemsetAsync(f.dMisc.p, 0, 64, ctx->st()));
        LAUNCH(ctx, "bg_active", k_active, dim3((unsigned)((P->d + 255) / 256)), dim3(256), 0, P->W.as<float>(), f.g,
               P->ring_dr.as<int>(), P->ring_dc.as<int>(), f.dAsum.as<float>(), f.dActive.as<unsigned char>(), f.dMisc.as<int>());
        CK(hipMemcpyAsync((char *)P->stat_host + 8, f.dMisc.p, sizeof(int), hipMemcpyDeviceToHost, ctx->st()));
        f.nactive = -1;
    }
    return fit_b0(f, f.g);
}
static int fit_pair_tables(RingFit &f) {
    cnmfe_ctx *ctx = f.ctx; Patch *P = f.P;
    f.npairs = plan::ring_pairs(P->nr_b, P->nc_b, P->roff, P->coff, P->nr, P->nc, f.reach.p_radius, f.reach.maxd, &f.pairs, &f.pair_of);
    plan::ring_tables(f.pairs, f.reach.maxd, f.reach.p_radius, P->dr.data(), P->dc.data(), P->p, f.tabs);
    f.nwork = (int)f.tabs.work.size();
    f.ht.mark("pair / need / work tables");
    RET(to_dev(ctx, f.dPairs, f.pairs)); RET(to_dev(ctx, f.dPairOf, f.pair_of)); RET(to_dev(ctx, f.dWork, f.tabs.work)); RET(to_dev(ctx, f.dNeed, f.tabs.needmask));
    const size_t cov_bytes = (size_t)f.npairs * BLKPX * BLKPX * sizeof(double);
    RET(ctx->cov.ensure(cov_bytes));
    if (ctx->opt("debug", 0)) CK(hipMemsetAsync(ctx->cov.p, 0xff, cov_bytes, ctx->st()));
    RET(to_dev(ctx, f.dTcnt, f.tabs.tcnt)); RET(to_dev(ctx, f.dTl, f.tabs.tlist));
    f.ht.mark("tile lists + uploads (sync)");
    if (f.incr) {
        RET(P->cov_base.ensure(cov_bytes));
        if (f.build_base && ctx->opt("debug", 0)) CK(hipMemsetAsync(P->cov_base.p, 0xff, cov_bytes, ctx->st()));
    }
    return 0;
}
static int fit_build_bf(RingFit &f, DevBuf &rsT) {
    cnmfe_ctx *ctx = f.ctx; Patch *P = f.P; const BgGeom &g = f.g; const int nblk = f.nblk;
    const bool has_a_bf = f.has_a && !f.incr;
    RET(ctx->bf.ensure((size_t)nblk * g.Tpad * BLKPX * sizeof(float))); RET(rsT.ensure((size_t)nblk * BLKPX * sizeof(double)));
    if (!f.use_i8) {
        const int tchunk = (int)((std::max<int64_t>(64, (g.Tpad + 15) / 16) + 7) & ~int64_t(7));
        LAUNCH(ctx, "bg_build_bf", k_build_bf, dim3(nblk, (unsigned)((g.Tpad + tchunk - 1) / tchunk)), dim3(256), 0, P->Yc4.as<float4>(), P->Tc, g,
               has_a_bf ? f.dArow.as<int>() : nullptr, f.dAcol.as<int>(), f.dAval.as<float>(), f.dCc.as<float>(), f.ldc, ctx->bf.as<float>(), tchunk, rsT.as<double>());
        return 0;
    }
    const size_t dbytes = (size_t)nblk * g.Tpad * BLKPX * sizeof(float), sbytes = (size_t)nblk * BLKPX * sizeof(double);
    bool resident = f.incr && planes_wanted(ctx, P, f.kstride);
    if (resident) RET(fits_leaving(P->dig, dbytes, &resident));
    if (resident) {
        RET(P->dig.ensure(dbytes)); RET(P->dig_sc.ensure(sbytes));
        f.digp = P->dig.as<uint4>(); f.digs = P->dig_sc.as<double>();
        P->dig_T16 = g.Tpad >> 4; P->dig_valid = true; P->digp_valid = false;
    } else {
        RET(ctx->dig_scale.ensure(sbytes));
        f.digp = ctx->bf.as<uint4>(); f.digs = ctx->dig_scale.as<double>();
    }
    int nchunk = 0;
    RET(build_digits(ctx, P, g, DigA{has_a_bf ? f.dArow.as<int>() : nullptr, f.dAcol.as<int>(), f.dAval.as<float>(), f.dCc.as<float>(), f.ldc}, f.digs, f.digp, &nchunk));
    LAUNCH(ctx, "bg_rs_reduce", k_rs_reduce, dim3((unsigned)nblk), dim3(256), 0, ctx->dig_rspart.as<double>(), nchunk, (int64_t)nblk * BLKPX, rsT.as<double>());
    if (f.incr && f.kstride > 1 && !has_a_bf && f.T <= (int64_t)I8_SEG_FRAMES * 16 && planes_wanted(ctx, P, 1)) {
        BgGeom g1 = g; g1.kstride = 1; geom_frames(g1, f.T, true);
        bool ok = false;
        RET(fits_leaving(P->dig, (size_t)nblk * g1.Tpad * BLKPX * sizeof(float), &ok));
        if (ok) {
            RET(P->dig.ensure((size_t)nblk * g1.Tpad * BLKPX * sizeof(float))); RET(P->dig_sc.ensure(sbytes));
            RET(build_digits(ctx, P, g1, DigA{nullptr, nullptr, nullptr, nullptr, 0}, P->dig_sc.as<double>(), P->dig.as<uint4>(), nullptr));
            P->dig_T16 = g1.Tpad >> 4; P->dig_valid = true; P->digp_valid = false;
        }
    }
    return 0;
}
static int fit_outlier_frames(RingFit &f) {
    cnmfe_ctx *ctx = f.ctx; Patch *P = f.P; BgGeom &g = f.g; const int64_t T = f.T;
    const size_t bfbytes = (size_t)f.nblk * g.Tpad * BLKPX * sizeof(float);
    RET(ctx->bf2.ensure(bfbytes)); RET(ctx->outl_cnt.ensure((size_t)T * sizeof(int)));
    CK(hipMemcpyAsync(ctx->bf2.p, ctx->bf.p, bfbytes, hipMemcpyDeviceToDevice, ctx->st()));
    CK(hipMemsetAsync(ctx->outl_cnt.p, 0, (size_t)T * sizeof(int), ctx->st()));
    LAUNCH(ctx, "bg_outlier_clip", k_outlier_clip, dim3((unsigned)((P->d + 255) / 256), (unsigned)(g.Tpad >> 2)), dim3(256), 0, ctx->bf.as<float4>(),
           ctx->bf2.as<float4>(), g, P->ring_dr.as<int>(), P->ring_dc.as<int>(), P->W.as<float>(), P->sn_b.as<float>(), f.thresh_outlier,
           ctx->outl_cnt.as<int>());
    std::vector<int> sel;
    const int64_t nmax = (int64_t)f.pmax * 100;
    if (nmax < T) {
        std::vector<int> cnt((size_t)T);
        CK(hipMemcpyAsync(cnt.data(), ctx->outl_cnt.p, (size_t)T * sizeof(int), hipMemcpyDeviceToHost, ctx->st()));
        CK(hipStreamSynchronize(ctx->st()));
        const double qv = matlab_quantile(cnt, (double)nmax / (double)T);
        for (int64_t t = 0; t < T; ++t) if ((double)cnt[t] <= qv) sel.push_back((int)t);
    } else for (int64_t t = 0; t < T; ++t) sel.push_back((int)t);
    const int64_t Tpad_src = g.Tpad;
    geom_frames(g, (int64_t)sel.size(), false);
    RET(to_dev(ctx, ctx->outl_sel, sel));
    LAUNCH(ctx, "bg_select_frames", k_select_frames, dim3(f.nblk, (unsigned)std::min<int64_t>(64, std::max<int64_t>(1, g.Tpad >> 2))), dim3(256), 0,
           ctx->bf2.as<float>(), Tpad_src, ctx->bf.as<float>(), g.Tpad, ctx->outl_sel.as<int>(), g.Tp);
    CK(hipStreamSynchronize(ctx->st()));
    return 0;
}
static int fit_base_table(RingFit &f) {
    cnmfe_ctx *ctx = f.ctx; Patch *P = f.P; const BgGeom &g = f.g;
    DevBuf &covT = f.incr ? P->cov_base : ctx->cov, &rsT = f.incr ? P->rowsum_base : ctx->rowsum;
    RET(fit_build_bf(f, rsT));
    if (f.outl) RET(fit_outlier_frames(f));
    if (g.bf4 < 2) LAUNCH(ctx, "bg_rowsum", k_rowsum, dim3(f.nblk), dim3(256), 0, ctx->bf.as<float>(), g.Tpad, rsT.as<double>(), g.bf4);
    const int nwg = (f.nwork + 7) / 8 * 8;
    const size_t shmem = (size_t)G4_NBUF * G4_STAGE_F * sizeof(float);
    static bool attr4 = false, attr8 = false;
    if (!attr4) { CK(hipFuncSetAttribute((const void *)k_gram4, hipFuncAttributeMaxDynamicSharedMemorySize, (int)shmem)); attr4 = true; }
    if (f.use_i8) {
        if (!attr8) { CK(hipFuncSetAttribute((const void *)k_gram_i8, hipFuncAttributeMaxDynamicSharedMemorySize, GI_NBUF * GI_STAGE_B)); attr8 = true; }
        LAUNCH(ctx, "bg_gram_i8", k_gram_i8, dim3(nwg), dim3(512), (size_t)GI_NBUF * GI_STAGE_B, f.digp, g.Tpad >> 4, f.dPairs.as<int4>(), f.dWork.as<int>(), f.nwork,
               f.dTcnt.as<int>(), f.dTl.as<int>(), f.digs, covT.as<double>());
    } else
        LAUNCH(ctx, "bg_gram_f64", k_gram4, dim3(nwg), dim3(256), shmem, ctx->bf.as<float>(), g.Tpad, f.dPairs.as<int4>(), f.dWork.as<int>(), f.nwork,
               f.dTcnt.as<int>(), f.dTl.as<int>(), 0, covT.as<double>());
    if (f.incr) { P->base_valid = true; P->base_kstride = f.kstride; }
    return 0;
}
static int fit_win_codes(RingFit &f) {
    const int woff = f.reach.woff, nwin = (f.g.nbr + 2 * woff) * (f.g.nbc + 2 * woff);
    RET(f.ctx->wcodes.ensure((size_t)nwin * 256 * sizeof(int)));
    LAUNCH(f.ctx, "bg_win_codes", k_win_codes, dim3((unsigned)nwin), dim3(256), 0, f.dPairOf.as<int>(), f.g.nbr, f.g.nbc, woff, f.reach.maxd, f.reach.nrel, f.ctx->wcodes.as<int>());
    return 0;
}
static int fit_pack(RingFit &f) {
    cnmfe_ctx *ctx = f.ctx; Patch *P = f.P; const int nt = f.nt;
    const double fillv[2] = {0.0, 1.0};
    RET(to_dev(ctx, ctx->solve_fill, fillv, 2));
    f.packed = f.incr && pack_wanted(ctx, nt) && (int64_t)f.nblk * std::max(1, f.K) < (int64_t)1 << 31 && (int64_t)f.L.lst_k.size() * BLKPX < (int64_t)1 << 31;
    const size_t sys_bytes = sys_bytes_of(P->d, nt);
    if (!f.packed || (P->sys_valid && P->sys.cap >= sys_bytes)) return 0;
    RET(fits_leaving(P->sys, sys_bytes, &f.packed));
    if (!f.packed) return 0;
    RET(P->sys.ensure(sys_bytes));
    RET(fit_win_codes(f));
    CovTab tb = f.covtab(); tb.cov = P->cov_base.as<double>(); tb.wcodes = ctx->wcodes.as<int>(); tb.woff = f.reach.woff;
    int *dErrP = nullptr;
    RET(ctx_errflag(ctx, &dErrP));
    RET(nt_dispatch<8>(nt, [&](auto c) -> int {
        LAUNCH(ctx, "bg_sys_pack", (k_sys_pack<NT_OF(c)>), dim3((unsigned)P->d), dim3(64), 0, tb, f.g, P->ring_dr.as<int>(), P->ring_dc.as<int>(), P->rowsum_base.as<double>(),
               (const unsigned char *)nullptr, (float *)nullptr, dErrP, 0, (const int *)nullptr, ctx->solve_fill.as<double>(), P->sys.as<double>());
        return 0; }));
    P->drop_inverses(); P->sys_valid = true;
    return 0;
}
static int fit_stage_windows(RingFit &f) {
    cnmfe_ctx *ctx = f.ctx; Patch *P = f.P;
    if (!(f.packed && ctx->opt("solve_staged", 1) != 0 && P->nr_b < 32768 && P->nc_b < 32768)) return 0;
    static thread_local std::vector<int> nmeta, lmeta;
    const int64_t tot = plan::stage_windows(f.K, fit_nbox, f.L.lst_k, P->nr_b, P->nc_b, f.reach.p_radius, nmeta, lmeta);
    if (tot < 0) return 0;
    f.stage_ok = true;
    RET(to_dev(ctx, ctx->stg[0], nmeta)); RET(to_dev(ctx, ctx->stg[1], lmeta));
    RET(ctx->stg[2].ensure((size_t)std::max<int64_t>(1, tot) * sizeof(double)));
    RET(ctx->stg[3].ensure((size_t)std::max<int64_t>(1, tot) * sizeof(float)));
    int *dErrW = nullptr;
    RET(ctx_errflag(ctx, &dErrW));
    LAUNCH(ctx, "bg_neuron_windows", k_nwin_build, dim3((unsigned)f.K), dim3(256), 0, ctx->stg[0].as<int>(), f.g, (int)f.K, f.dArow.as<int>(), f.dAcol.as<int>(), f.dAval.as<float>(),
           f.dLp->as<int>(), f.dSlot->as<short>(), f.dUt.as<double>(), ctx->stg[2].as<double>(), ctx->stg[3].as<float>(), dErrW);
    return 0;
}
static int fit_corrections(RingFit &f, const float *C, int c_order) {
    cnmfe_ctx *ctx = f.ctx; Patch *P = f.P; const BgGeom &g = f.g; const int K = (int)f.K;
    RET(ctx->rowsum.ensure((size_t)f.nblk * BLKPX * sizeof(double)));
    if (!f.has_a) {
        if (!f.packed) CK(hipMemcpyAsync(ctx->cov.p, P->cov_base.p, (size_t)f.npairs * BLKPX * BLKPX * sizeof(double), hipMemcpyDeviceToDevice, ctx->st()));
        CK(hipMemcpyAsync(ctx->rowsum.p, P->rowsum_base.p, (size_t)f.nblk * BLKPX * sizeof(double), hipMemcpyDeviceToDevice, ctx->st()));
        return 0;
    }
    if (!f.proj_queued) RET(fit_queue_projection(f));
    RET(to_dev(ctx, *f.dSlot, f.L.slot_of));
    if (f.keep_pt) RET(P->pt_tab.ensure(std::max<size_t>(1, f.L.lst_k.size()) * BLKPX * sizeof(double)));
    LAUNCH(ctx, "bg_win_fix", k_win_fix, dim3((unsigned)f.L.blall.size(), WIN_NLB / WF_S), dim3(256), 0, g, K, f.dArow.as<int>(), f.dAcol.as<int>(), f.dAval.as<float>(), f.dLp->as<int>(),
           f.dSlot->as<short>(), f.dBl.as<int>(), f.nsg, f.dUt.as<double>(), f.ut_stride, f.dGb.as<double>(), f.gb_stride, f.keep_pt ? P->pt_tab.as<double>() : nullptr,
           f.win_i8 ? ctx->gk.as<double>() : (const double *)nullptr, f.dLk.as<int>());
    if (f.keep_pt) {
        P->pt_K = K; P->pt_lp_h = f.L.lst_ptr; P->pt_slot_h = f.L.slot_of;
        P->pt_gen = bound_rows_of(ctx, C, c_order, K, P->pt_rows) ? ctx->bound_gen : -1;
        P->pt_valid = true;
    }
    const int csplit = f.npairs >= 8192 ? 1 : f.npairs >= 4096 ? 2 : 4;
    if (!f.packed)
        LAUNCH(ctx, "bg_cov_correct", k_cov_correct, dim3((unsigned)f.npairs, (unsigned)csplit), dim3(256), 0, P->cov_base.as<double>(), ctx->cov.as<double>(), f.dPairs.as<int4>(),
               f.dNeed.as<unsigned short>(), g, K, f.dArow.as<int>(), f.dAcol.as<int>(), f.dAval.as<float>(), f.dLp->as<int>(), f.dSlot->as<short>(), f.dUt.as<double>());
    LAUNCH(ctx, "bg_rowsum_correct", k_rowsum_correct, dim3(f.nblk), dim3(256), 0, P->rowsum_base.as<double>(), ctx->rowsum.as<double>(), g,
           f.dArow.as<int>(), f.dAcol.as<int>(), f.dAval.as<float>(), f.dCsum.as<double>());
    return fit_stage_windows(f);
}
static int fit_solve_packed(RingFit &f, const unsigned char *act, int probe) {
    cnmfe_ctx *ctx = f.ctx; Patch *P = f.P; const BgGeom &g = f.g; const int nt = f.nt;
    const int *dr = P->ring_dr.as<int>(), *dc = P->ring_dc.as<int>(); const double *sys = P->sys.as<double>(), *rowsum = ctx->rowsum.as<double>(); float *W = P->W.as<float>();
    const unsigned d = (unsigned)P->d;
    PackArgs pa{};
    if (f.has_a) {
        pa.arow = f.dArow.as<int>(); pa.acol = f.dAcol.as<int>(); pa.aval = f.dAval.as<float>(); pa.lst_ptr = f.dLp->as<int>(); pa.lst_k = f.dLk.as<int>();
        pa.slot_of = f.dSlot->as<short>(); pa.K = (int)f.K; pa.Ut = f.dUt.as<double>();
    }
    int *dErrS = nullptr;
    RET(ctx_errflag(ctx, &dErrS));
    const int inv_mode = (int)ctx->opt("solve_inv", 0);
    const size_t kinv_bytes = (size_t)P->d * (size_t)ri_stride(nt) * sizeof(double);
    bool inv_ok = inv_mode != 0 && f.has_a && nt <= 6 && !(probe & 7);
    if (inv_ok) RET(fits_leaving(P->kinv, kinv_bytes, &inv_ok));
    double *lam_arr = nullptr;
    if (inv_ok) {
        if (P->kinv_lam.cap < (size_t)P->d * sizeof(double)) { RET(P->kinv_lam.ensure((size_t)P->d * sizeof(double))); P->kinv_lam_valid = false; }
        RET(P->kinv_list.ensure(((size_t)2 * P->d + 4) * sizeof(int)));
        if (!P->kinv_lam_valid) { CK(hipMemsetAsync(P->kinv_lam.p, 0, (size_t)P->d * sizeof(double), ctx->st())); P->kinv_lam_valid = true; }
        lam_arr = P->kinv_lam.as<double>();
        if (!P->kinv_valid && (P->kinv_fits >= 1 || inv_mode >= 2)) {
            RET(P->kinv.ensure(kinv_bytes));
            RET(nt_dispatch<6>(nt, [&](auto c) -> int {
                LAUNCH(ctx, "bg_ring_inverse", (k_ring_inverse<NT_OF(c)>), dim3(d), dim3(64), 0, sys, g, dr, dc, P->rowsum_base.as<double>(), (const double *)lam_arr, P->kinv.as<double>());
                return 0; }));
            P->kinv_valid = true;
        }
        ++P->kinv_fits;
    }
    if (inv_ok && P->kinv_valid) {
        int *flist = P->kinv_list.as<int>(), *rlist = flist + P->d, *fcnt = flist + 2 * P->d;
        CK(hipMemsetAsync(fcnt, 0, 4 * sizeof(int), ctx->st()));
        InvArgs ia{};
        ia.kp = P->kinv.as<double>(); ia.sys = P->sys.as<double>(); ia.csum = f.dCsum.as<double>(); ia.lam_out = lam_arr;
        ia.flist = flist; ia.rlist = rlist; ia.fcnt = fcnt; ia.maxit = (int)ctx->opt("solve_inv_terms", 5);
        const unsigned nlist = (unsigned)std::min<int64_t>(P->d, 2048);
        return nt_dispatch<6>(nt, [&](auto c) -> int {
            LAUNCH(ctx, "bg_ring_solve", (k_ring_apply<NT_OF(c)>), dim3(d), dim3(64), 0, ia, pa, g, dr, dc, rowsum, act, W, dErrS, probe, (const int *)nullptr);
            LAUNCH(ctx, "bg_ring_solve_rest", (k_ring_solve6<NT_OF(c)>), dim3(d), dim3(64), 0, sys, pa, g, dr, dc, rowsum, (const unsigned char *)nullptr, W, dErrS, probe, (const int *)flist,
                   (const int *)fcnt, lam_arr);
            LAUNCH(ctx, "bg_ring_inverse_rest", (k_ring_inverse_list<NT_OF(c)>), dim3(nlist), dim3(64), 0, sys, g, dr, dc, P->rowsum_base.as<double>(), (const double *)lam_arr,
                   P->kinv.as<double>(), (const int *)rlist, (const int *)(fcnt + 3));
            return 0; });
    }
    if (f.has_a && f.stage_ok && nt <= 6) {
        StageArgs sg{f.dLp->as<int>(), ctx->stg[1].as<int>(), ctx->stg[2].as<double>(), ctx->stg[3].as<float>()};
        return nt_dispatch<6>(nt, [&](auto c) -> int {
            LAUNCH(ctx, "bg_ring_solve", (k_ring_solve8<NT_OF(c)>), dim3(d), dim3(64), 0, sys, sg, g, dr, dc, rowsum, act, W, dErrS, probe, (const int *)nullptr, lam_arr);
            return 0; });
    }
    return nt_dispatch<8>(nt, [&](auto c) -> int {
        LAUNCH(ctx, "bg_ring_solve", (k_ring_solve6<NT_OF(c)>), dim3(d), dim3(64), 0, sys, pa, g, dr, dc, rowsum, act, W, dErrS, probe, (const int *)nullptr, (const int *)nullptr, lam_arr);
        return 0; });
}
static int fit_solve(RingFit &f) {
    cnmfe_ctx *ctx = f.ctx;
    const unsigned char *act = f.first_run ? nullptr : f.dActive.as<unsigned char>();
    const int probe = (int)ctx->opt("solve_probe", 0);
    if (f.packed) return fit_solve_packed(f, act, probe);
    RET(fit_win_codes(f));
    CovTab tab = f.covtab(); tab.wcodes = ctx->wcodes.as<int>(); tab.woff = f.reach.woff;
    return solve_launch(ctx, f.P, tab, f.g, ctx->rowsum.as<double>(), act, f.nt, probe, ctx->solve_fill.as<double>());
}

int bg_fit_ring(cnmfe_ctx *ctx, Patch *P, int32_t K, const int64_t *A_colptr, const int32_t *A_rowidx, const float *A_val,
                const float *C, int c_order, int with_projection, float *b0_out, int64_t info[4], int b0_only, double thresh_outlier) {
    RingFit f(ctx, P);
    f.K = K; f.A_colptr = A_colptr; f.A_rowidx = A_rowidx; f.A_val = A_val; f.C = C; f.c_order = c_order; f.b0_only = b0_only; f.thresh_outlier = thresh_outlier; f.T = P->T;
    f.outl = thresh_outlier == thresh_outlier; f.has_a = K > 0 && A_colptr[K] > 0; f.a_empty = K == 0;
    if (f.outl && !P->sn_ready && !(b0_only & 1)) return fail(CNMFE_ESTATE, "fit_ring_model with thresh_outlier needs the noise levels of the block (cnmfe_set_noise)");
    RET(fit_traces_up(f));
    f.ht.mark("traces");
    if (b0_only & 1) {
        RET(fit_upload_csr(f));
        RET(fit_b0(f, bg_geom(P)));
        P->ysig_valid = false;
        return 0;
    }
    RET(fit_geometry(f, with_projection));
    fit_lists(f);
    if (f.incr && f.has_a && !f.build_base) RET(fit_queue_projection(f));
    f.ht.mark("projection queued");
    RET(fit_upload_csr(f));
    f.ht.mark("A csr");
    RET(fit_active_b0(f));
    f.ht.mark("ind_active + b0");
    RET(fit_pair_tables(f));
    if (!f.incr || f.build_base) RET(fit_base_table(f));
    if (f.nt < 1 || f.nt > 8) return fail(CNMFE_EUNSUPPORTED, "fit_ring_model: %d ring neighbours (<= %d supported)", P->p, PMAX_RING);
    RET(fit_pack(f));
    if (f.incr) RET(fit_corrections(f, C, c_order));
    f.ht.mark("base / correction launches");
    RET(fit_solve(f));
    RET(ring_stats_enqueue(ctx, P));
    f.ht.mark("solve launch");
    if (b0_out) {
        std::vector<double> tmp(P->d);
        CK(hipMemcpyAsync(tmp.data(), P->b0.p, P->d * sizeof(double), hipMemcpyDeviceToHost, ctx->st()));
        CK(hipStreamSynchronize(ctx->st()));
        for (int64_t i = 0; i < P->d; ++i) b0_out[i] = (float)tmp[i];
        if (f.nactive < 0) f.nactive = *reinterpret_cast<const int *>((const char *)P->stat_host + 8);
    }
    if (info) { info[0] = f.first_run ? 1 : 0; info[1] = f.kstride; info[2] = f.nactive; info[3] = f.pmax; }
    P->ysig_valid = false;
    return 0;
}

int win_i8_table(cnmfe_ctx *ctx, Patch *P, const char *name_dig, const char *name_proj, int K, const float *dCc, int64_t ldc, const std::vector<int> &lst_ptr, const std::vector<int> &blall,
                 const int *dLp, const int *dLk, int nsg, double *dUt, int64_t ut_stride) {
    RET(trace_digits(ctx, name_dig, dCc, ldc, K, P->T, P->dig_T16, false));
    return win_proj_i8_launch(ctx, P, name_proj, lst_ptr, blall, dLp, dLk, nsg, dUt, ut_stride);
}

int tu_warm_bg() { hipFuncAttributes at; return hipFuncGetAttributes(&at, (const void *)k_rowsum) == hipSuccess ? 0 : -1; }

}
```

### cnmf_e_amd/csrc/common.hpp

```cpp
#pragma once
#include <hip/hip_runtime.h>
#include <stdint.h>
#include <stdio.h>
#include <stdarg.h>
#include <string.h>
#include <string>
#include <vector>
#include <cstring>
#include <chrono>
#include <cmath>
#include <map>
#include <algorithm>
#include "../../include/cnmfe.h"

namespace cnmfe {

typedef unsigned nt_u32x4_t __attribute__((ext_vector_type(4)));
__device__ __forceinline__ uint4 ld_stream(const uint4 *p) {
    const nt_u32x4_t v = __builtin_nontemporal_load(reinterpret_cast<const nt_u32x4_t *>(p));
    return make_uint4(v.x, v.y, v.z, v.w);
}


extern thread_local char g_err[1024];
inline int fail(int code, const char *fmt, ...) {
    va_list ap; va_start(ap, fmt); vsnprintf(g_err, sizeof(g_err), fmt, ap); va_end(ap);
    return code;
}

#define CK(call) do { hipError_t e_ = (call); if (e_ != hipSuccess) \
    return cnmfe::fail(CNMFE_EHIP, "%s:%d %s -> %s", __FILE__, __LINE__, #call, hipGetErrorString(e_)); } while (0)
#define RET(x) do { int r_ = (x); if (r_ != 0) return r_; } while (0)

void pin_flush_all();
void pin_flush_range(const void *p, size_t bytes);

struct DevBuf {
    void *p = nullptr; size_t cap = 0;
    ~DevBuf() { if (p) { pin_flush_range(p, cap); (void)hipFree(p); } }
    DevBuf() = default;
    DevBuf(const DevBuf &) = delete; DevBuf &operator=(const DevBuf &) = delete;
    int ensure(size_t bytes) {
        if (bytes <= cap) return 0;
        const size_t grown = (p && bytes < (size_t(64) << 20)) ? std::max(bytes, cap + cap / 2) : bytes;
        static const bool trace_alloc_ = getenv("CNMFE_TRACE_ALLOC") != nullptr;
        if (trace_alloc_ && p) fprintf(stderr, "[alloc] grow %zu -> %zu bytes (hipFree + hipMalloc)\n", cap, grown);
        if (p) { pin_flush_range(p, cap); (void)hipFree(p); p = nullptr; cap = 0; }
        size_t want = (grown + 255) & ~size_t(255);
        hipError_t e = hipMalloc(&p, want);
        if (e != hipSuccess) { p = nullptr; return fail(CNMFE_ENOMEM, "hipMalloc(%zu) failed: %s", want, hipGetErrorString(e)); }
        cap = want; return 0;
    }
    int ensure_hw(size_t bytes, size_t &hw) { if (bytes > hw) hw = bytes; return ensure(hw); }
    template <class T> T *as() const { return reinterpret_cast<T *>(p); }
    void swap(DevBuf &o) { std::swap(p, o.p); std::swap(cap, o.cap); }
};

struct Profiler {
    int on = 0;
    static bool selected(const char *n) {
        static const char *const sel[] = {"residual_r1", "bg_ring_solve", "bg_win_proj", "bg_cov_correct", "spatial_proj_U", "temporal_proj_U"};
        for (const char *s : sel) if (!strcmp(n, s)) return true;
        return false;
    }
    bool want(const char *n) const { return on == 1 || (on == 2 && selected(n)); }
    struct Rec { hipEvent_t a, b; int id; };
    std::vector<std::string> names;
    std::vector<double> total_ms; std::vector<int64_t> calls;
    std::vector<Rec> pending;
    std::vector<hipEvent_t> pool;
    int id_of(const char *n) {
        for (size_t i = 0; i < names.size(); ++i) if (names[i] == n) return (int)i;
        names.push_back(n); total_ms.push_back(0); calls.push_back(0); return (int)names.size() - 1;
    }
    hipEvent_t ev() { if (!pool.empty()) { hipEvent_t e = pool.back(); pool.pop_back(); return e; }
                      hipEvent_t e; (void)hipEventCreate(&e); return e; }
    void begin(const char *n, hipStream_t s, Rec &r) { r.id = id_of(n); r.a = ev(); r.b = ev(); (void)hipEventRecord(r.a, s); }
    void end(hipStream_t s, Rec &r) { (void)hipEventRecord(r.b, s); pending.push_back(r); }
    void drain() {
        for (auto &r : pending) {
            (void)hipEventSynchronize(r.b); float ms = 0; (void)hipEventElapsedTime(&ms, r.a, r.b);
            total_ms[r.id] += ms; calls[r.id] += 1; pool.push_back(r.a); pool.push_back(r.b);
        }
        pending.clear();
    }
    void reset() { drain(); for (auto &t : total_ms) t = 0; for (auto &c : calls) c = 0; }
    ~Profiler() { drain(); for (auto e : pool) (void)hipEventDestroy(e); }
};

#define LAUNCH(ctx, name, kern, grid, block, shmem, ...) do { \
    cnmfe::Profiler::Rec pr_; bool pon_ = (ctx)->prof.on && (ctx)->prof.want(name); \
    const bool ltr_ = (ctx)->trace_level >= 2; \
    const auto lt0_ = ltr_ ? std::chrono::steady_clock::now() : std::chrono::steady_clock::time_point(); \
    hipStream_t lst_ = (ctx)->st(); \
    if (pon_) (ctx)->prof.begin(name, lst_, pr_); \
    const auto lt1_ = ltr_ ? std::chrono::steady_clock::now() : std::chrono::steady_clock::time_point(); \
    hipLaunchKernelGGL(kern, grid, block, shmem, lst_, __VA_ARGS__); \
    if (ltr_) { const auto lt2_ = std::chrono::steady_clock::now(); const double la_ = std::chrono::duration<double, std::milli>(lt1_ - lt0_).count(), lb_ = std::chrono::duration<double, std::milli>(lt2_ - lt1_).count(); \
        if (la_ + lb_ > 2.0) fprintf(stderr, "[host_trace] launch %s: flush of held-back uploads %.2f ms, launch call %.2f ms\n", name, la_, lb_); } \
    if (pon_) (ctx)->prof.end(lst_, pr_); \
    hipError_t le_ = hipGetLastError(); \
    if (le_ != hipSuccess) return cnmfe::fail(CNMFE_EHIP, "launch %s failed: %s", name, hipGetErrorString(le_)); \
} while (0)

constexpr int PMAX_RING = 128;
constexpr int BLK = 16;
constexpr int BLKPX = BLK * BLK;

struct HostCSR { std::vector<int32_t> rowptr;    std::vector<int32_t> col; std::vector<float> val; std::vector<int32_t> src; };
inline void csc_to_csr(int64_t nrow, int32_t ncol, const int64_t *colptr, const int32_t *rowidx, const float *val, HostCSR &out) {
    int64_t nnz = colptr[ncol];
    out.rowptr.assign(nrow + 1, 0); out.col.resize(nnz); out.val.resize(nnz); out.src.resize(nnz);
    for (int64_t e = 0; e < nnz; ++e) out.rowptr[rowidx[e] + 1]++;
    for (int64_t r = 0; r < nrow; ++r) out.rowptr[r + 1] += out.rowptr[r];
    std::vector<int32_t> cur(out.rowptr.begin(), out.rowptr.end() - 1);
    for (int32_t k = 0; k < ncol; ++k)
        for (int64_t e = colptr[k]; e < colptr[k + 1]; ++e) {
            int32_t pos = cur[rowidx[e]]++; out.col[pos] = k; out.val[pos] = val ? val[e] : 1.0f; out.src[pos] = (int32_t)e;
        }
}

struct PeelSession { DevBuf hy, yw, sn, q, ci, scr; int64_t n = 0, nq = 0; int M = 0; int64_t d = 0; int nr = 0, nc = 0; bool residual = false; };
struct SeedSrc { const float4 *y4; int64_t d; int nr, nc; };

struct Patch {
    int32_t prect[4], brect[4];
    int32_t d1 = 0, d2 = 0;
    int32_t nr = 0, nc = 0, nr_b = 0, nc_b = 0;
    int32_t roff = 0, coff = 0;
    int64_t T = 0, d = 0, d_b = 0;
    DevBuf Y;
    DevBuf Yc4;
    int64_t Tc = 0;
    DevBuf ymean_d;
    DevBuf ymean_f;
    bool ymean_valid = false;
    int64_t frames_uploaded = 0;
    std::vector<uint8_t> frame_seen;
    int32_t radius = 0, p = 0;
    std::vector<int32_t> dr, dc;
    DevBuf ring_dr, ring_dc;
    DevBuf W;
    DevBuf b0;
    bool ring_ready = false;
    DevBuf sn_b;
    bool sn_ready = false;
    DevBuf ysig;
    bool ysig_valid = false;
    bool ysig_virtual = false;
    DevBuf pt_tab, pt_lp, pt_slot;
    bool pt_valid = false; int32_t pt_K = 0; int64_t pt_gen = -1;
    std::vector<int32_t> pt_rows; std::vector<int> pt_lp_h; std::vector<short> pt_slot_h;
    int64_t res_gen = 0;
    bool res_ac = false; int res_kind = 0; int64_t res_ldc = 0;
    DevBuf resCnt, resK, resV, resCc, resCm;
    bool pend = false, pend_ac = false; int64_t pend_ldc = 0; int32_t pend_K = 0, res_K = 0;
    DevBuf pendCnt, pendK, pendV, pendCc, pendCm;
    DevBuf cov_base, rowsum_base;
    bool base_valid = false, derived = false;
    int base_kstride = 0;
    DevBuf cov_base_alt, rowsum_base_alt; bool base_alt_valid = false; int base_alt_kstride = 0;
    DevBuf sys, sys_alt; bool sys_valid = false, sys_alt_valid = false;
    DevBuf kinv, kinv_lam, kinv_list; bool kinv_valid = false, kinv_lam_valid = false; int kinv_fits = 0;
    void drop_inverses() { kinv_valid = false; kinv_lam_valid = false; kinv_fits = 0; }
    void drop_systems() { sys_valid = false; drop_inverses(); }
    DevBuf dig, dig_sc; int64_t dig_T16 = 0; bool dig_valid = false;
    DevBuf yt4; bool yt4_valid = false;
    DevBuf digp; bool digp_valid = false;
    int ss_res = -1, ss_ssub = 0, ss_Pr = 0, ss_Pc = 0, ss_d1s = 0, ss_d2s = 0;
    bool ss_taps = false;
    std::vector<int> ss_tr_idx, ss_tc_idx, ss_rlo, ss_rhi, ss_clo, ss_chi, ss_trp_h, ss_tri_h, ss_tcp_h, ss_tci_h;
    std::vector<float> ss_tr_w, ss_tc_w;
    DevBuf ss_ir, ss_wr, ss_ic, ss_wc, ss_trp, ss_tri, ss_trw, ss_tcp, ss_tci, ss_tcw, ss_dlt;
    DevBuf stat_dev; void *stat_host = nullptr; hipEvent_t stat_ev = nullptr; bool stat_valid = false;
    int lane = 0;
    PeelSession *peel = nullptr;
    ~Patch() { delete peel; if (stat_host) (void)hipHostFree(stat_host); if (stat_ev) (void)hipEventDestroy(stat_ev); }
};

struct DeconvScratch { DevBuf pv, pw, pt, pl, tkp, tko, tkl, tkv, pnum, list, ybuf, obuf, tbuf;
    void swap(DeconvScratch &o) { DevBuf *a[] = {&pv, &pw, &pt, &pl, &tkp, &tko, &tkl, &tkv, &pnum, &list, &ybuf, &obuf, &tbuf}, *b[] = {&o.pv, &o.pw, &o.pt, &o.pl, &o.tkp, &o.tko, &o.tkl, &o.tkv, &o.pnum, &o.list, &o.ybuf, &o.obuf, &o.tbuf};
        for (int i = 0; i < 13; ++i) a[i]->swap(*b[i]); } };

struct TemporalJob {
    Patch *P = nullptr; int32_t K = 0; int64_t ldc = 0, T = 0; int maxIter = 0; bool deconv = false; cnmfe_deconv_opts dopts{};
    DevBuf dC, dColptr, dErow, dAval, dU, dCraw, dNk, dNidx, dNval, dNptr, dAa, dOvf, dS, dPars, dSn, dB;
    std::vector<std::vector<int>> levels;
    bool swept = false;
    bool dag = false;
    std::vector<int> diag; std::vector<char> upd; bool term_applied = false, finished = false; int nn = 0;
    float *pin = nullptr; size_t pin_cap = 0;
    ~TemporalJob() { if (pin) (void)hipHostFree(pin); }
};

}

namespace cnmfe {
struct PinArena {
    char *p = nullptr; size_t cap = 0, off = 0; int half = 0;
    hipEvent_t ev[2] = {nullptr, nullptr}; bool ev_set[2] = {false, false};
    int init(size_t bytes) {
        if (p) return 0;
        if (hipHostMalloc((void **)&p, bytes, hipHostMallocDefault) != hipSuccess) { p = nullptr; return -1; }
        cap = bytes;
        for (int i = 0; i < 2; ++i) if (hipEventCreateWithFlags(&ev[i], hipEventDisableTiming) != hipSuccess) return -1;
        return 0;
    }
    template <class F> void *take(size_t n, F &&stream_of) {
        n = (n + 255) & ~size_t(255);
        if (!p || n > cap / 2) return nullptr;
        const size_t end = (size_t)(half + 1) * (cap / 2);
        if (off + n > end) {
            (void)hipEventRecord(ev[half], stream_of()); ev_set[half] = true;
            half ^= 1; off = (size_t)half * (cap / 2);
            if (ev_set[half]) (void)hipEventSynchronize(ev[half]);
        }
        void *r = p + off; off += n; return r;
    }
    void swap(PinArena &o) { std::swap(p, o.p); std::swap(cap, o.cap); std::swap(off, o.off); std::swap(half, o.half); for (int i = 0; i < 2; ++i) { std::swap(ev[i], o.ev[i]); std::swap(ev_set[i], o.ev_set[i]); } }
    ~PinArena() { if (p) (void)hipHostFree(p); for (int i = 0; i < 2; ++i) if (ev[i]) (void)hipEventDestroy(ev[i]); }
};
}

namespace cnmfe {
constexpr int PIN_NSEG = 24;
constexpr int I8_SEG_FRAMES = 24576;
struct PinSegs { const uint4 *src[PIN_NSEG]; uint4 *dst[PIN_NSEG]; unsigned n16[PIN_NSEG]; };
}

struct cnmfe_lane {
    hipStream_t stream_ = nullptr; cnmfe::PinSegs pseg{}; int npseg = 0; cnmfe::PinArena pin; int64_t spatial_nnz = -1;
    cnmfe::DevBuf vp[32]; size_t hw_vp[32] = {}; int64_t last_ldc = 0;
    cnmfe::DevBuf ysig_low, up_tmp, bgs_r, bgs_b, bgs_upr, bgs_upc; int bgs_patch = -1, bgs_d1s = 0; int64_t bgs_dF = 0;
    cnmfe::DevBuf bf, dig_smax, dig_rspart, dig_scale, tdig, tscale, gk, win_items, bf2, outl_cnt, outl_sel, cov, rowsum, tmp[16];
    size_t hw_cc = 0, hw_cm = 0, hw_wa[3] = {0, 0, 0};
    cnmfe::DevBuf inc[7], stg[4], wcodes, solve_fill, stage, scr[24]; cnmfe::DeconvScratch dscr;
    hipEvent_t ev = nullptr; int64_t fork_seen = 0; bool dirty = false;
    ~cnmfe_lane() { if (stream_) (void)hipStreamDestroy(stream_); if (ev) (void)hipEventDestroy(ev); }
};

struct cnmfe_ctx {
    int device = 0;
    hipStream_t stream_ = nullptr;
    cnmfe::PinSegs pseg; int npseg = 0;
    void flush_copies();
    hipStream_t st() { if (npseg) flush_copies(); return stream_; }
    cnmfe::PinArena pin;
    int64_t spatial_nnz = -1;
    hipStream_t copy_stream = nullptr;
    hipEvent_t ev_bound_ready = nullptr, ev_copy_done = nullptr; bool copy_pending = false;
    int64_t copy_gen = 0; std::vector<std::pair<int64_t, hipEvent_t>> copy_gens; std::vector<hipEvent_t> copy_ev_pool;
    int copy_batch_mark();
    std::vector<hipEvent_t> tickets; std::vector<char> ticket_busy;
    int *ticket_flags = nullptr;
    cnmfe::DevBuf ticket_dev;
    static constexpr size_t TICKET_FLAGS = 1024;
    cnmfe::Profiler prof;
    std::map<int, cnmfe::Patch *> patches;
    cnmfe::DevBuf bound;
    int32_t bound_K = 0; int64_t bound_T = 0; int bound_order = 1; bool bound_valid = false;
    int64_t bound_gen = 0;
    cnmfe::DevBuf vp[32];
    size_t hw_vp[32] = {};
    int64_t last_ldc = 0;
    cnmfe::DevBuf ysig_low;
    cnmfe::DevBuf up_tmp;
    cnmfe::DevBuf bgs_r, bgs_b, bgs_upr, bgs_upc;
    int bgs_patch = -1, bgs_d1s = 0; int64_t bgs_dF = 0;
    cnmfe::DevBuf bf;
    cnmfe::DevBuf dig_smax;
    cnmfe::DevBuf dig_rspart;
    cnmfe::DevBuf dig_scale;
    cnmfe::DevBuf tdig, tscale, gk, win_items;
    cnmfe::DevBuf bf2, outl_cnt, outl_sel;
    cnmfe::DevBuf cov;
    cnmfe::DevBuf rowsum;
    cnmfe::DevBuf tmp[16];
    size_t hw_cc = 0, hw_cm = 0, hw_wa[3] = {0, 0, 0};
    cnmfe::DevBuf inc[7];
    cnmfe::DevBuf stg[4];
    cnmfe::DevBuf wcodes, solve_fill;
    cnmfe::DevBuf stage;
    cnmfe::DevBuf scr[24];
    cnmfe::DeconvScratch dscr;
    cnmfe::DevBuf last_craw, last_aa;
    struct EarlyU {
        bool valid = false; int64_t token = 0, claimed = 0;
        cnmfe::Patch *P = nullptr; int32_t K = 0; int64_t ldc = 0, T = 0, spatial_gen = 0, res_gen = 0;
        int64_t proj_i8 = 0, proj_i8_planes = 0, proj_tiled = 0;
    } early;
    cnmfe::DevBuf early_a, early_u;
    cnmfe::Patch *spatial_patch = nullptr; int32_t spatial_K = 0;
    int64_t spatial_gen = 0, conn_gen = -1;
    int64_t last_nent = 0;
    int64_t early_seq = 0, early_hits = 0, early_drops = 0, early_declined = 0, early_nent = 0, sweep_nowait = 0;
    std::vector<cnmfe::TemporalJob *> tjobs; int tjobs_used = 0;
    cnmfe::DevBuf dcv_c, dcv_s, dcv_pars, dcv_sn;
    int64_t res_gen = -1; bool res_has_s = false;
    cnmfe::DevBuf mrg[23];
    int32_t diff_K = 0; int64_t diff_T = 0;
    int64_t merge_uploads = 0;
    int32_t last_t_K = 0; int64_t last_t_ldc = 0, last_t_T = 0; bool last_t_valid = false;
    cnmfe::DevBuf stitch;
    int32_t stitch_K = 0; int64_t stitch_T = 0, stitch_ld = 0; bool stitch_open = false;
    void *rccl_comm = nullptr; int rccl_rank = 0, rccl_n = 0;
    cnmfe::DevBuf errflag;
    std::map<std::string, int64_t> opts;
    int trace_level = 0;
    int64_t opt(const char *n, int64_t dflt) const { auto it = opts.find(n); return it == opts.end() ? dflt : it->second; }
    std::vector<cnmfe_lane *> lanes; int cur_lane = 0, patches_created = 0, spatial_lane = 0;
    hipEvent_t ev_fork = nullptr; int64_t fork_gen = 0;
    void swap_lane(cnmfe_lane &L);
    int activate(int lane);
    int join_lanes();
    int fork_mark();
    ~cnmfe_ctx();
};

namespace cnmfe {
struct HostTrace {
    bool on; const char *name; std::chrono::steady_clock::time_point t0, last;
    HostTrace(cnmfe_ctx *ctx, const char *n) : on(ctx->opt("host_trace", 0) != 0), name(n) { if (on) t0 = last = std::chrono::steady_clock::now(); }
    void mark(const char *what) {
        if (!on) return;
        const auto t = std::chrono::steady_clock::now();
        fprintf(stderr, "[host_trace] %s: %-28s %8.3f ms (at %8.3f)\n", name, what, std::chrono::duration<double, std::milli>(t - last).count(),
                std::chrono::duration<double, std::milli>(t - t0).count());
        last = t;
    }
};
inline Patch *get_patch(cnmfe_ctx *ctx, int id) {
    auto it = ctx->patches.find(id);
    if (it == ctx->patches.end()) return nullptr;
    if (!ctx->lanes.empty() && ctx->activate(it->second->lane) != 0) return nullptr;
    return it->second;
}
struct GlobalScope {
    cnmfe_ctx *ctx; int rc = 0;
    explicit GlobalScope(cnmfe_ctx *c) : ctx(c) { if (ctx && !ctx->lanes.empty()) rc = ctx->join_lanes(); }
    ~GlobalScope() { if (ctx && !ctx->lanes.empty()) (void)ctx->fork_mark(); }
};
int pinned_to_dev(cnmfe_ctx *ctx, void *dst, const void *src_pinned, size_t bytes);
void pin_register(cnmfe_ctx *ctx, bool live);
template <class T> inline int to_dev(cnmfe_ctx *ctx, DevBuf &b, const T *h, size_t n) {
    RET(b.ensure(std::max<size_t>(n, 1) * sizeof(T)));
    if (!n) return 0;
    if (void *st = ctx->pin.take(n * sizeof(T), [ctx] { return ctx->st(); })) {
        memcpy(st, h, n * sizeof(T));
        return pinned_to_dev(ctx, b.p, st, n * sizeof(T));
    }
    CK(hipMemcpyAsync(b.p, h, n * sizeof(T), hipMemcpyHostToDevice, ctx->st()));
    CK(hipStreamSynchronize(ctx->st()));
    return 0;
}
template <class T> inline int to_dev(cnmfe_ctx *ctx, DevBuf &b, const std::vector<T> &h) { return to_dev(ctx, b, h.data(), h.size()); }
int upload_traces(cnmfe_ctx *ctx, DevBuf &dst, const float *C, int32_t K, int64_t T, int order, int64_t *ldc);
int download_traces(cnmfe_ctx *ctx, const float *dC, int64_t ldc, float *C, int32_t K, int64_t T, int order);

int bg_fit_ring(cnmfe_ctx *ctx, Patch *P, int32_t K, const int64_t *A_colptr, const int32_t *A_rowidx, const float *A_val,
                const float *C, int c_order, int with_projection, float *b0_out, int64_t info[4], int b0_only = 0, double thresh_outlier = NAN);
int tu_warm_resid(); int tu_warm_bg();
int win_i8_table(cnmfe_ctx *ctx, Patch *P, const char *name_dig, const char *name_proj, int K, const float *dCc, int64_t ldc, const std::vector<int> &lst_ptr, const std::vector<int> &blall,
                 const int *dLp, const int *dLk, int nsg, double *dUt, int64_t ut_stride);
int tu_warm_factor(); int tu_warm_deconv(); int tu_warm_ssub(); int tu_warm_vproj();
int fits_leaving(const DevBuf &b, size_t bytes, bool *fits, bool quarter = false);
int bg_reserve(cnmfe_ctx *ctx, Patch *P);
int residual_run(cnmfe_ctx *ctx, Patch *P, int pid, int32_t Ksel, const int64_t *A_colptr, const int32_t *A_rowidx,
                 const float *A_val, const float *C, int c_order, float *Ysig_out, int out_memspace, DevBuf *outbuf = nullptr, int tables_only = 0);
int ysig_export(cnmfe_ctx *ctx, Patch *P, DevBuf &ysig, float *Ysig_out, int out_memspace);
int rss_run(cnmfe_ctx *ctx, Patch *P, int32_t K, const int64_t *A_colptr, const int32_t *A_rowidx, const float *A_val, const float *C, int c_order,
            const float *b0_block, const float *b0_new, double *rss_out);
int bg_reconstruct_run(cnmfe_ctx *ctx, Patch *P, const float *b0_block, const float *b0_new, int64_t frame0, int64_t nframes, float *out, int out_memspace);
int residual_materialize(cnmfe_ctx *ctx, Patch *P);
int residual_realize(cnmfe_ctx *ctx, Patch *P);
bool bound_rows_of(const cnmfe_ctx *ctx, const float *C, int c_order, int32_t K, std::vector<int32_t> &rows);
int vproj_spatial(cnmfe_ctx *ctx, Patch *P, int32_t K, const float *C, int c_order, const int64_t *IND_colptr, const int32_t *IND_rowidx,
                  const int *dErow, const int *dEcol, const float *dCc, int64_t ldc, float *dU, double *dQ = nullptr);
int vproj_temporal(cnmfe_ctx *ctx, Patch *P, int32_t K, const int64_t *A_colptr, const int32_t *A_rowidx, const float *A_val,
                   const int64_t *dColptr, const int *dErow, const float *dAval, float *dU, int64_t ldu);
int vproj_spatial_ssub(cnmfe_ctx *ctx, Patch *M, int32_t K, const float *C, int c_order, const int64_t *IND_colptr, const int32_t *IND_rowidx,
                       const int *dErow, const int *dEcol, const float *dCc, int64_t ldc, float *dU);
int vproj_temporal_ssub(cnmfe_ctx *ctx, Patch *M, int32_t K, const int64_t *A_colptr, const int32_t *A_rowidx, const float *A_val,
                        const int64_t *dColptr, const int *dErow, const float *dAval, float *dU, int64_t ldu);
int ssub_taps(cnmfe_ctx *ctx, Patch *M, const Patch *R);
int ssub_realize(cnmfe_ctx *ctx, Patch *M);
int residual_term_project(cnmfe_ctx *ctx, Patch *P, int32_t K, const int64_t *dColptr, const int *dErow, const float *dAval, float *dU, int64_t ldu, int *dOverflow);
bool residual_term_foldable_spatial(const Patch *P, int32_t K, int64_t ldc);
int residual_term_fold_spatial(cnmfe_ctx *ctx, Patch *P, int32_t K, int64_t nnz, const int *dErow, const int *dEcol, const float *dCc, int64_t ldc, float *dU, DevBuf &dG);
int check_csc_pub(const char *what, int32_t ncol, int64_t nrow, const int64_t *colptr, const int32_t *rowidx);
int spatial_run(cnmfe_ctx *ctx, Patch *P, int algorithm, int32_t K, const int64_t *A_colptr, const int32_t *A_rowidx,
                const float *A_val, const float *C, int c_order, const int64_t *IND_colptr, const int32_t *IND_rowidx,
                const float *sn, int32_t param, float *A_out);
int temporal_run(cnmfe_ctx *ctx, Patch *P, int32_t K, const int64_t *A_colptr, const int32_t *A_rowidx, const float *A_val,
                 const float *C_in, int c_order, int32_t maxIter, float *C_out, float *C_raw_out, float *aa_out,
                 const cnmfe_deconv_opts *dopts, float *kernel_pars, float *S_out, float *sn_out, TemporalJob *job = nullptr);
int temporal_sweep_jobs(cnmfe_ctx *ctx);
#ifdef __HIPCC__
__device__ __forceinline__ void glds16(const void *base, unsigned voff, unsigned lds_dst) {
    unsigned keep;
    asm volatile("s_mov_b32 %0, m0\n\ts_mov_b32 m0, %3\n\ts_nop 0\n\tglobal_load_lds_dwordx4 %1, %2\n\ts_mov_b32 m0, %0"
                 : "=&s"(keep) : "v"(voff), "s"(base), "s"(lds_dst) : "memory");
}
#endif

int sn_pixels_run(cnmfe_ctx *ctx, Patch *P, float *sn_out);
int fast_temporal_run(cnmfe_ctx *ctx, Patch *P, int32_t K, const int64_t *A_colptr, const int32_t *A_rowidx, const float *A_val,
                      int c_order, float *C_raw_out, float *aa_out);
int deconv_bound_run(cnmfe_ctx *ctx, const cnmfe_deconv_opts *opts, float *C_out, float *C_raw_out, float *S_out, float *pars_out, float *sn_out);
int deconv_all_run(cnmfe_ctx *ctx, int32_t K, int64_t T, float *C_raw, int c_order, const cnmfe_deconv_opts *opts,
                   float *C_out, float *S_out, float *pars_out, float *sn_out);
int trace_corr_run(cnmfe_ctx *ctx, int32_t K, int64_t T, const float *X, int src, int raw, double *out);
int trace_diff_spikes_run(cnmfe_ctx *ctx, int32_t K, int64_t T, const float *X, int src, float *sn_out, float *S_out);
int trace_tags_run(cnmfe_ctx *ctx, int32_t K, double *out);
int traces_load_run(cnmfe_ctx *ctx, int32_t K, int64_t T, const float *C, const float *C_raw, const float *S, const float *pars, int c_order);
int merge_apply_run(cnmfe_ctx *ctx, int32_t ng, const int32_t *gptr, const int32_t *gidx, const double *w, int32_t nkeep, const int32_t *keep,
                    const cnmfe_deconv_opts *opts, float *C_out, float *C_raw_out, float *S_out, float *pars_out, float *sn_out);
int postproc_run(cnmfe_ctx *ctx, int32_t d1, int32_t d2, int32_t K, const int64_t *A_colptr, const int32_t *A_rowidx,
                 const float *A_val, uint8_t *keep);
int ensure_ymean(cnmfe_ctx *ctx, Patch *P);
int sn_video_run(cnmfe_ctx *ctx, Patch *P, int64_t nframes, float *sn_out);
int seed_images_run(cnmfe_ctx *ctx, const SeedSrc &src, const float *psf, int32_t psf_n, int64_t nframes, const double *Q, int32_t M, float sig,
                    float *Cn_out, float *PNR_out, PeelSession *keep = nullptr);
int peel_open_residual_run(cnmfe_ctx *ctx, Patch *P, int32_t Ksel, const int64_t *A_colptr, const int32_t *A_rowidx, const float *A_val, const float *C, int c_order,
                           const float *psf, int32_t psf_n, float sig, float *Cn_out, float *PNR_out, float *Sn_out, float *Yres_out, int out_memspace);
int peel_open_run(cnmfe_ctx *ctx, Patch *P, const float *psf, int32_t psf_n, int64_t nframes, const double *Q, int32_t M, float sig,
                  float *Cn_out, float *PNR_out, float *Sn_out);
int peel_extract_run(cnmfe_ctx *ctx, Patch *P, int r, int c, int gSiz, double *corr_box, double *ai_box, double *ci_out, double *stats);
int peel_apply_run(cnmfe_ctx *ctx, Patch *P, int r, int c, int gSiz, const double *ai_box, const double *Hai_box2, const double *ci, double sig, double min_pnr,
                   double min_corr, float *PNR_box2, float *Cn_box2);
int spatial_fetch(cnmfe_ctx *ctx, float *A_out, int64_t nnz);
int spatial_fetch_connected(cnmfe_ctx *ctx, int32_t d1, int32_t d2, int32_t K, const int64_t *IND_colptr, const int32_t *IND_rowidx, float *A_out, uint8_t *keep, bool wait = true);
int temporal_early_project(cnmfe_ctx *ctx, int32_t K, const int64_t *IND_colptr, const int32_t *IND_rowidx, int64_t *token);
int ring_first_run(cnmfe_ctx *ctx, Patch *P, bool *first);
int ring_stats_enqueue(cnmfe_ctx *ctx, Patch *P);
int ring_stats_get(cnmfe_ctx *ctx, Patch *P, int *pmax, bool *first);
int center_traces(cnmfe_ctx *ctx, const float *C, int64_t ldc, int32_t K, int64_t T, DevBuf &Cc, DevBuf &Cmean);
int upload_centered(cnmfe_ctx *ctx, DevBuf &stage, const float *C, int32_t K, int64_t T, int order, DevBuf &Cc, DevBuf &Cmean, int64_t *ldc_out);
int ctx_errflag(cnmfe_ctx *ctx, int **dflag);
int ctx_check_errflag(cnmfe_ctx *ctx);
}
```

Measured before the change: 98.83 iter/s.

## Overlap ring-fit setup on side stream, cache pair tables, move A row sums to GPU

Measured after the change: 101.2 iter/s, median of 6. +2.4%, better.

```diff
diff --git a/cnmf_e_amd/csrc/api.hip b/cnmf_e_amd/csrc/api.hip
--- a/cnmf_e_amd/csrc/api.hip
+++ b/cnmf_e_amd/csrc/api.hip
@@ -308,6 +308,24 @@
 }
 
 int ring_first_run(cnmfe_ctx *ctx, Patch *P, bool *first) { return ring_stats_get(ctx, P, nullptr, first); }
+int ctx_side_stream(cnmfe_ctx *ctx) {
+    if (ctx->side_stream) return 0;
+    int prio = 0;
+    CK(hipStreamGetPriority(ctx->stream_, &prio));
+    hipStream_t s = nullptr;
+    CK(hipStreamCreateWithPriority(&s, hipStreamDefault, prio));
+    hipLaunchKernelGGL(k_scratch_warm, dim3(1), dim3(64), 0, s, (int *)nullptr, 3);
+    hipError_t e = hipStreamSynchronize(s);
+    if (e == hipSuccess) e = hipEventCreateWithFlags(&ctx->ev_side_fork, hipEventDisableTiming);
+    if (e == hipSuccess) e = hipEventCreateWithFlags(&ctx->ev_side_join, hipEventDisableTiming);
+    if (e != hipSuccess) {
+        (void)hipStreamDestroy(s);
+        if (ctx->ev_side_fork) { (void)hipEventDestroy(ctx->ev_side_fork); ctx->ev_side_fork = nullptr; }
+        return fail(CNMFE_EHIP, "side stream of option fit_side: %s", hipGetErrorString(e));
+    }
+    ctx->side_stream = s;
+    return 0;
+}
 int ctx_errflag(cnmfe_ctx *ctx, int **dflag) {
     if (!ctx->errflag.p) {
         RET(ctx->errflag.ensure(sizeof(int)));
@@ -573,6 +591,9 @@
     (void)hipSetDevice(ctx->device);
     (void)ctx->join_lanes();
     (void)hipStreamSynchronize(ctx->st());
+    if (ctx->side_stream) { (void)hipStreamSynchronize(ctx->side_stream); (void)hipStreamDestroy(ctx->side_stream); ctx->side_stream = nullptr; }
+    if (ctx->ev_side_fork) { (void)hipEventDestroy(ctx->ev_side_fork); ctx->ev_side_fork = nullptr; }
+    if (ctx->ev_side_join) { (void)hipEventDestroy(ctx->ev_side_join); ctx->ev_side_join = nullptr; }
     delete ctx;
 }
 
@@ -586,7 +607,7 @@
 
 int cnmfe_set_option(cnmfe_ctx *ctx, const char *name, int64_t value) {
     if (!ctx || !name) return fail(CNMFE_EINVAL, "null argument");
-    static const char *known[] = {"r1_variant", "r1_delta", "r1_lazy", "r1_defer", "r1_virtual", "gram_incremental", "prealloc", "solve_packed", "sweep_dag", "win_i8_planes", "solve_staged", "solve_inv", "solve_inv_terms", "gram_i8", "win_i8", "proj_tiled", "proj_i8", "proj_i8_planes", "ssub_virtual", "temporal_early",
+    static const char *known[] = {"r1_variant", "r1_delta", "r1_lazy", "r1_defer", "r1_virtual", "gram_incremental", "prealloc", "solve_packed", "sweep_dag", "win_i8_planes", "solve_staged", "solve_inv", "solve_inv_terms", "gram_i8", "win_i8", "proj_tiled", "proj_i8", "proj_i8_planes", "ssub_virtual", "temporal_early", "fit_side",
                                   "solve_probe", "r1_probe", "deconv_trace", "host_trace", "debug", nullptr};
     if (!strcmp(name, "lanes")) { RET(lanes_set(ctx, value)); ctx->opts[name] = value; return 0; }
     for (int i = 0; known[i]; ++i) if (!strcmp(known[i], name)) { ctx->opts[name] = value; if (!strcmp(name, "host_trace")) ctx->trace_level = (int)value; return 0; }
diff --git a/cnmf_e_amd/csrc/bg.hip b/cnmf_e_amd/csrc/bg.hip
--- a/cnmf_e_amd/csrc/bg.hip
+++ b/cnmf_e_amd/csrc/bg.hip
@@ -433,6 +433,19 @@
 #include "win_proj_i8.hpp"
 namespace cnmfe {
 
+__global__ void __launch_bounds__(256) k_asum(const int *__restrict__ arow, const float *__restrict__ aval, float fillv, int64_t n, float *__restrict__ asum) {
+    const int64_t q = (int64_t)blockIdx.x * blockDim.x + threadIdx.x;
+    if (q >= n) return;
+    if (!arow) { asum[q] = fillv; return; }
+    double s = 0;
+    for (int e = arow[q]; e < arow[q + 1]; ++e) s += aval[e];
+    asum[q] = (float)s;
+}
+__global__ void __launch_bounds__(64) k_slot_build(const int *__restrict__ lst_ptr, const int *__restrict__ lst_k, int K, short *__restrict__ slot_of) {
+    const int b = blockIdx.x, p0 = lst_ptr[b], n = lst_ptr[b + 1] - p0;
+    for (int s = threadIdx.x; s < n; s += blockDim.x) slot_of[(int64_t)b * K + lst_k[p0 + s]] = (short)s;
+}
+
 __global__ void k_active(const float *__restrict__ W, BgGeom g, const int *__restrict__ dr, const int *__restrict__ dc,
                          const float *__restrict__ asum, unsigned char *__restrict__ active, int *__restrict__ nactive) {
     int64_t m = (int64_t)blockIdx.x * blockDim.x + threadIdx.x;
@@ -550,25 +563,37 @@
 static bool pack_wanted(cnmfe_ctx *ctx, int nt) { return ctx->opt("solve_packed", 1) != 0 && nt >= 1 && nt <= 8; }
 static size_t sys_bytes_of(int64_t d, int nt) { return (size_t)d * ((size_t)(nt * (nt + 1) / 2) * 256 + 16 * nt) * sizeof(double); }
 
+static int trace_gram(cnmfe_ctx *ctx, const float *dCc, int64_t ldc, int K, int64_t T) {
+    RET(ctx->gk.ensure((size_t)K * K * sizeof(double)));
+    LAUNCH(ctx, "bg_trace_gram", k_trace_gram, dim3((unsigned)(((K + 15) >> 4) * (((K + 15) >> 4) + 1) / 2)), dim3(64 * TG_W), 0, dCc, ldc, T, K, ctx->gk.as<double>());
+    return 0;
+}
 static int trace_digits(cnmfe_ctx *ctx, const char *name, const float *dCc, int64_t ldc, int K, int64_t T, int64_t T16, bool gram) {
     RET(ctx->tdig.ensure((size_t)K * T16 * 4 * sizeof(uint4))); RET(ctx->tscale.ensure((size_t)K * sizeof(double)));
     if (gram) RET(ctx->gk.ensure((size_t)K * K * sizeof(double)));
     LAUNCH(ctx, name, k_trace_dig, dim3(K), dim3(256), 0, dCc, ldc, T, T16, ctx->tdig.as<uint4>(), ctx->tscale.as<double>());
-    if (gram) LAUNCH(ctx, "bg_trace_gram", k_trace_gram, dim3((unsigned)(((K + 15) >> 4) * (((K + 15) >> 4) + 1) / 2)), dim3(64 * TG_W), 0, dCc, ldc, T, K, ctx->gk.as<double>());
-    return 0;
-}
-static int win_proj_i8_launch(cnmfe_ctx *ctx, Patch *P, const char *name, const std::vector<int> &lst_ptr, const std::vector<int> &blall, const int *dLp, const int *dLk, int nsg,
-                              double *dUt, int64_t ut_stride) {
+    return gram ? trace_gram(ctx, dCc, ldc, K, T) : 0;
+}
+static int win_proj_i8_items(cnmfe_ctx *ctx, const std::vector<int> &lst_ptr, const std::vector<int> &blall, size_t *nitems) {
     static thread_local std::vector<int> items;
     plan::win_i8_items(blall, lst_ptr, items);
-    RET(to_dev(ctx, ctx->win_items, items));
-    if (items.empty()) return 0;
+    *nitems = items.size();
+    return to_dev(ctx, ctx->win_items, items);
+}
+static int win_proj_i8_go(cnmfe_ctx *ctx, Patch *P, const char *name, size_t nitems, const int *dLp, const int *dLk, int nsg, double *dUt, int64_t ut_stride) {
+    if (!nitems) return 0;
     const int64_t T16 = P->dig_T16;
-#define WPI8_GO(V0_) LAUNCH(ctx, name, k_win_proj_i8<V0_>, dim3((unsigned)(items.size() * nsg)), dim3(512), 0, P->dig.as<uint4>(), T16, P->dig_sc.as<double>(), ctx->tdig.as<uint4>(), \
+#define WPI8_GO(V0_) LAUNCH(ctx, name, k_win_proj_i8<V0_>, dim3((unsigned)(nitems * nsg)), dim3(512), 0, P->dig.as<uint4>(), T16, P->dig_sc.as<double>(), ctx->tdig.as<uint4>(), \
                             ctx->tscale.as<double>(), dLp, dLk, ctx->win_items.as<int>(), nsg, dUt, ut_stride)
     if (win_planes3(ctx, T16)) WPI8_GO(1); else WPI8_GO(0);
 #undef WPI8_GO
     return 0;
+}
+static int win_proj_i8_launch(cnmfe_ctx *ctx, Patch *P, const char *name, const std::vector<int> &lst_ptr, const std::vector<int> &blall, const int *dLp, const int *dLk, int nsg,
+                              double *dUt, int64_t ut_stride) {
+    size_t nitems = 0;
+    RET(win_proj_i8_items(ctx, lst_ptr, blall, &nitems));
+    return win_proj_i8_go(ctx, P, name, nitems, dLp, dLk, nsg, dUt, ut_stride);
 }
 static int build_digits(cnmfe_ctx *ctx, Patch *P, const BgGeom &g, const DigA &da, double *digs, uint4 *digp, int *nchunk) {
     const int nblk = g.nbr * g.nbc;
@@ -618,13 +643,14 @@
     HostCSR csr;
     bool first_run = false; int pmax = 0, kstride = 1;
     BgGeom g; plan::Reach reach; int nblk = 0, nt = 0;
-    plan::BlockLists L; std::vector<plan::Pair> pairs; std::vector<int> pair_of; plan::Tables tabs; int npairs = 0, nwork = 0;
+    plan::BlockLists L; int npairs = 0, nwork = 0;
     bool incr = false, build_base = false, use_i8 = false, keep_pt = false, trace_i8_done = false, proj_queued = false, win_i8 = false, packed = false, stage_ok = false;
+    bool gram_pending = false, setup_done = false, stage_planned = false; int64_t stage_tot = -1;
     int nsg = 1; int64_t ut_stride = 0, gb_stride = 0;
     uint4 *digp = nullptr; double *digs = nullptr;
     DevBuf &dC, &dCc, &dCm, &dArow, &dAcol, &dAval, &dMisc, &dAsum, &dActive, &dPairs, &dPairOf, &dWork, &dNeed, &dTcnt, &dTl, &dLk, &dBl, &dUt, &dCsum, &dGb, *dLp, *dSlot;
     RingFit(cnmfe_ctx *c, Patch *p_) : ctx(c), P(p_), ht(c, "fit_ring"), dC(c->tmp[0]), dCc(c->tmp[1]), dCm(c->tmp[2]), dArow(c->tmp[3]), dAcol(c->tmp[4]), dAval(c->tmp[5]), dMisc(c->tmp[6]),
-        dAsum(c->tmp[7]), dActive(c->tmp[8]), dPairs(c->tmp[9]), dPairOf(c->tmp[10]), dWork(c->tmp[11]), dNeed(c->tmp[7]), dTcnt(c->tmp[12]), dTl(c->tmp[13]), dLk(c->inc[1]),
+        dAsum(c->tmp[7]), dActive(c->tmp[8]), dPairs(p_->rt.dPairs), dPairOf(p_->rt.dPairOf), dWork(p_->rt.dWork), dNeed(p_->rt.dNeed), dTcnt(p_->rt.dTcnt), dTl(p_->rt.dTl), dLk(c->inc[1]),
         dBl(c->inc[3]), dUt(c->inc[4]), dCsum(c->inc[5]), dGb(c->inc[6]), dLp(&c->inc[0]), dSlot(&c->inc[2]) {}
     const int *arow() const { return has_a ? dArow.as<int>() : nullptr; }
     CovTab covtab() const { CovTab t{}; t.cov = ctx->cov.as<double>(); t.pair_of = dPairOf.as<int>(); t.nbr = g.nbr; t.nbc = g.nbc; t.maxd = reach.maxd; t.nrel = reach.nrel; return t; }
@@ -636,10 +662,16 @@
     if (!f.has_a) return 0;
     RET(upload_centered(ctx, f.dC, f.C, f.K, f.T, f.c_order, f.dCc, f.dCm, &f.ldc));
     if (!f.outl && ctx->opt("gram_incremental", 1) != 0 && win_i8_applies(ctx, P, P->base_valid ? P->base_kstride : 1)) {
-        RET(trace_digits(ctx, "bg_trace_dig", f.dCc.as<float>(), f.ldc, f.K, f.T, P->dig_T16, true));
+        f.gram_pending = ctx->opt("fit_side", 1) != 0 && ctx->lanes.empty();
+        RET(trace_digits(ctx, "bg_trace_dig", f.dCc.as<float>(), f.ldc, f.K, f.T, P->dig_T16, !f.gram_pending));
         f.trace_i8_done = true;
     }
     return 0;
+}
+static int fit_trace_gram(RingFit &f) {
+    if (!f.gram_pending) return 0;
+    f.gram_pending = false;
+    return trace_gram(f.ctx, f.dCc.as<float>(), f.ldc, f.K, f.T);
 }
 static int fit_upload_csr(RingFit &f) {
     if (!f.has_a) return 0;
@@ -685,25 +717,62 @@
     f.keep_pt = f.incr && f.has_a && f.kstride == 1 && !P->derived && !(f.b0_only & 2) && ctx->opt("r1_virtual", 1) != 0;
     if (f.keep_pt) { f.dLp = &P->pt_lp; f.dSlot = &P->pt_slot; P->pt_valid = false; }
 }
-static int fit_queue_projection(RingFit &f) {
+struct SideScope {
+    cnmfe_ctx *ctx; bool inside = false;
+    explicit SideScope(cnmfe_ctx *c) : ctx(c) {}
+    int fork() {
+        int *dErr = nullptr;
+        RET(ctx_errflag(ctx, &dErr));
+        RET(ctx_side_stream(ctx));
+        CK(hipEventRecord(ctx->ev_side_fork, ctx->st()));
+        CK(hipStreamWaitEvent(ctx->side_stream, ctx->ev_side_fork, 0));
+        return 0;
+    }
+    int enter() { (void)ctx->st(); std::swap(ctx->stream_, ctx->side_stream); inside = true; return 0; }
+    int leave() {
+        if (!inside) return 0;
+        const hipError_t e = hipEventRecord(ctx->ev_side_join, ctx->st());
+        std::swap(ctx->stream_, ctx->side_stream); inside = false;
+        CK(e);
+        CK(hipStreamWaitEvent(ctx->stream_, ctx->ev_side_join, 0));
+        return 0;
+    }
+    ~SideScope() { if (inside) (void)leave(); }
+};
+static int fit_side_mode(const RingFit &f) {
+    const int64_t m = f.ctx->opt("fit_side", 1);
+    return (m == 1 || m == 2) && f.ctx->lanes.empty() && f.incr && f.has_a && !f.build_base ? (int)m : 0;
+}
+static int fit_side_setup(RingFit &f);
+
+static int fit_queue_projection(RingFit &f, int side = 0) {
     cnmfe_ctx *ctx = f.ctx; Patch *P = f.P; const BgGeom &g = f.g;
+    SideScope sc(ctx);
     RET(to_dev(ctx, *f.dLp, f.L.lst_ptr)); RET(to_dev(ctx, f.dLk, f.L.lst_k)); RET(to_dev(ctx, f.dBl, f.L.blall)); RET(f.dCsum.ensure((size_t)f.K * sizeof(double)));
-    LAUNCH(ctx, "bg_trace_subsum", k_trace_subsum, dim3(f.K), dim3(256), 0, f.dCc.as<float>(), f.ldc, g.Tp, g.kstride, f.dCsum.as<double>());
+    if (!side) LAUNCH(ctx, "bg_trace_subsum", k_trace_subsum, dim3(f.K), dim3(256), 0, f.dCc.as<float>(), f.ldc, g.Tp, g.kstride, f.dCsum.as<double>());
     const int nb_ = (int)f.L.blall.size(), nbig = (int)f.L.blk_nt[3].size();
     f.nsg = plan::win_segments(nb_);
     f.ut_stride = (int64_t)std::max<size_t>(1, f.L.lst_k.size()) * BLKPX; f.gb_stride = (int64_t)f.nblk * WIN_NLB * WIN_NLB;
     RET(f.dUt.ensure((size_t)f.nsg * f.ut_stride * sizeof(double))); RET(f.dGb.ensure((size_t)f.nsg * f.gb_stride * sizeof(double)));
     const int *dLp = f.dLp->as<int>(), *dLk = f.dLk.as<int>(), *dBl = f.dBl.as<int>();
-    if (win_i8_applies(ctx, P, g.kstride)) {
-        if (!f.trace_i8_done) RET(trace_digits(ctx, "bg_trace_dig", f.dCc.as<float>(), f.ldc, f.K, f.T, P->dig_T16, true));
-        RET(win_proj_i8_launch(ctx, P, "bg_win_proj", f.L.lst_ptr, f.L.blall, dLp, dLk, f.nsg, f.dUt.as<double>(), f.ut_stride));
-        f.win_i8 = true;
+    f.win_i8 = win_i8_applies(ctx, P, g.kstride);
+    size_t nitems = 0;
+    if (f.win_i8) {
+        if (!f.trace_i8_done) { f.gram_pending = side != 0; RET(trace_digits(ctx, "bg_trace_dig", f.dCc.as<float>(), f.ldc, f.K, f.T, P->dig_T16, !f.gram_pending)); f.trace_i8_done = true; }
+        if (!side) RET(fit_trace_gram(f));
+        RET(win_proj_i8_items(ctx, f.L.lst_ptr, f.L.blall, &nitems));
+    }
+    if (side) RET(sc.fork());
+    if (side == 2) { RET(sc.enter()); RET(fit_side_setup(f)); RET(sc.leave()); }
+    if (f.win_i8) {
+        RET(win_proj_i8_go(ctx, P, "bg_win_proj", nitems, dLp, dLk, f.nsg, f.dUt.as<double>(), f.ut_stride));
     } else if (g.kstride == 1 || g.kstride == 2 || g.kstride == 4)
         RET(win_proj4_launch(ctx, "bg_win_proj", P, g, f.dCc.as<float>(), f.ldc, dLp, dLk, dBl, nbig, nb_, f.nsg, f.dUt.as<double>(), f.ut_stride, f.dGb.as<double>(), f.gb_stride));
     else
         LAUNCH(ctx, "bg_win_proj", k_win_proj, dim3((unsigned)(nb_ * f.nsg)), dim3(256), 0, P->Yc4.as<float4>(), g, f.dCc.as<float>(), f.ldc, dLp, dLk, dBl, f.nsg, f.dUt.as<double>(), f.ut_stride,
                f.dGb.as<double>(), f.gb_stride);
     f.proj_queued = true;
+    if (side == 1) { RET(sc.enter()); RET(fit_side_setup(f)); RET(sc.leave()); }
     return 0;
 }
 static int fit_active_b0(RingFit &f) {
@@ -711,10 +780,10 @@
     RET(f.dActive.ensure(P->d));
     f.nactive = P->d;
     if (f.first_run) { CK(hipMemsetAsync(f.dActive.p, 1, P->d, ctx->st())); } else {
-        std::vector<float> asum(P->d_b, 0.f);
-        if (f.a_empty || (f.b0_only & 2)) std::fill(asum.begin(), asum.end(), 1.0f);
-        else if (f.has_a) for (int64_t q = 0; q < P->d_b; ++q) { double s = 0; for (int64_t e = f.csr.rowptr[q]; e < f.csr.rowptr[q + 1]; ++e) s += f.csr.val[e]; asum[q] = (float)s; }
-        RET(to_dev(ctx, f.dAsum, asum));
+        const bool ones = f.a_empty || (f.b0_only & 2);
+        RET(f.dAsum.ensure((size_t)P->d_b * sizeof(float)));
+        LAUNCH(ctx, "bg_asum", k_asum, dim3((unsigned)((P->d_b + 255) / 256)), dim3(256), 0, !ones && f.has_a ? f.dArow.as<int>() : (const int *)nullptr, f.dAval.as<float>(), ones ? 1.0f : 0.0f,
+               (int64_t)P->d_b, f.dAsum.as<float>());
         CK(hipMemsetAsync(f.dMisc.p, 0, 64, ctx->st()));
         LAUNCH(ctx, "bg_active", k_active, dim3((unsigned)((P->d + 255) / 256)), dim3(256), 0, P->W.as<float>(), f.g,
                P->ring_dr.as<int>(), P->ring_dc.as<int>(), f.dAsum.as<float>(), f.dActive.as<unsigned char>(), f.dMisc.as<int>());
@@ -725,20 +794,36 @@
 }
 static int fit_pair_tables(RingFit &f) {
     cnmfe_ctx *ctx = f.ctx; Patch *P = f.P;
-    f.npairs = plan::ring_pairs(P->nr_b, P->nc_b, P->roff, P->coff, P->nr, P->nc, f.reach.p_radius, f.reach.maxd, &f.pairs, &f.pair_of);
-    plan::ring_tables(f.pairs, f.reach.maxd, f.reach.p_radius, P->dr.data(), P->dc.data(), P->p, f.tabs);
-    f.nwork = (int)f.tabs.work.size();
+    Patch::RingTabs &rt = P->rt;
+    const int geo[8] = {(int)P->nr_b, (int)P->nc_b, (int)P->roff, (int)P->coff, (int)P->nr, (int)P->nc, f.reach.p_radius, f.reach.maxd};
+    if (!(rt.keyed && std::equal(geo, geo + 8, rt.geo) && rt.dr == P->dr && rt.dc == P->dc)) {
+        rt.keyed = rt.built = false;
+        rt.npairs = plan::ring_pairs(geo[0], geo[1], geo[2], geo[3], geo[4], geo[5], geo[6], geo[7], nullptr, nullptr);
+        std::copy(geo, geo + 8, rt.geo); rt.dr = P->dr; rt.dc = P->dc; rt.keyed = true;
+    }
+    f.npairs = rt.npairs;
     f.ht.mark("pair / need / work tables");
-    RET(to_dev(ctx, f.dPairs, f.pairs)); RET(to_dev(ctx, f.dPairOf, f.pair_of)); RET(to_dev(ctx, f.dWork, f.tabs.work)); RET(to_dev(ctx, f.dNeed, f.tabs.needmask));
     const size_t cov_bytes = (size_t)f.npairs * BLKPX * BLKPX * sizeof(double);
     RET(ctx->cov.ensure(cov_bytes));
     if (ctx->opt("debug", 0)) CK(hipMemsetAsync(ctx->cov.p, 0xff, cov_bytes, ctx->st()));
-    RET(to_dev(ctx, f.dTcnt, f.tabs.tcnt)); RET(to_dev(ctx, f.dTl, f.tabs.tlist));
     f.ht.mark("tile lists + uploads (sync)");
     if (f.incr) {
         RET(P->cov_base.ensure(cov_bytes));
         if (f.build_base && ctx->opt("debug", 0)) CK(hipMemsetAsync(P->cov_base.p, 0xff, cov_bytes, ctx->st()));
     }
+    return 0;
+}
+static int fit_need_tables(RingFit &f) {
+    cnmfe_ctx *ctx = f.ctx; Patch *P = f.P; Patch::RingTabs &rt = P->rt;
+    if (!rt.built) {
+        plan::ring_pairs(rt.geo[0], rt.geo[1], rt.geo[2], rt.geo[3], rt.geo[4], rt.geo[5], rt.geo[6], rt.geo[7], &rt.pairs, &rt.pair_of);
+        plan::ring_tables(rt.pairs, f.reach.maxd, f.reach.p_radius, P->dr.data(), P->dc.data(), P->p, rt.tabs);
+        rt.nwork = (int)rt.tabs.work.size();
+        RET(to_dev(ctx, rt.dPairs, rt.pairs)); RET(to_dev(ctx, rt.dPairOf, rt.pair_of)); RET(to_dev(ctx, rt.dWork, rt.tabs.work)); RET(to_dev(ctx, rt.dNeed, rt.tabs.needmask));
+        RET(to_dev(ctx, rt.dTcnt, rt.tabs.tcnt)); RET(to_dev(ctx, rt.dTl, rt.tabs.tlist));
+        rt.built = true;
+    }
+    f.nwork = rt.nwork;
     return 0;
 }
 static int fit_build_bf(RingFit &f, DevBuf &rsT) {
@@ -806,6 +891,7 @@
 static int fit_base_table(RingFit &f) {
     cnmfe_ctx *ctx = f.ctx; Patch *P = f.P; const BgGeom &g = f.g;
     DevBuf &covT = f.incr ? P->cov_base : ctx->cov, &rsT = f.incr ? P->rowsum_base : ctx->rowsum;
+    RET(fit_need_tables(f));
     RET(fit_build_bf(f, rsT));
     if (f.outl) RET(fit_outlier_frames(f));
     if (g.bf4 < 2) LAUNCH(ctx, "bg_rowsum", k_rowsum, dim3(f.nblk), dim3(256), 0, ctx->bf.as<float>(), g.Tpad, rsT.as<double>(), g.bf4);
@@ -825,6 +911,7 @@
 }
 static int fit_win_codes(RingFit &f) {
     const int woff = f.reach.woff, nwin = (f.g.nbr + 2 * woff) * (f.g.nbc + 2 * woff);
+    RET(fit_need_tables(f));
     RET(f.ctx->wcodes.ensure((size_t)nwin * 256 * sizeof(int)));
     LAUNCH(f.ctx, "bg_win_codes", k_win_codes, dim3((unsigned)nwin), dim3(256), 0, f.dPairOf.as<int>(), f.g.nbr, f.g.nbc, woff, f.reach.maxd, f.reach.nrel, f.ctx->wcodes.as<int>());
     return 0;
@@ -832,7 +919,7 @@
 static int fit_pack(RingFit &f) {
     cnmfe_ctx *ctx = f.ctx; Patch *P = f.P; const int nt = f.nt;
     const double fillv[2] = {0.0, 1.0};
-    RET(to_dev(ctx, ctx->solve_fill, fillv, 2));
+    if (!ctx->solve_fill.p) RET(to_dev(ctx, ctx->solve_fill, fillv, 2));
     f.packed = f.incr && pack_wanted(ctx, nt) && (int64_t)f.nblk * std::max(1, f.K) < (int64_t)1 << 31 && (int64_t)f.L.lst_k.size() * BLKPX < (int64_t)1 << 31;
     const size_t sys_bytes = sys_bytes_of(P->d, nt);
     if (!f.packed || (P->sys_valid && P->sys.cap >= sys_bytes)) return 0;
@@ -850,20 +937,49 @@
     P->drop_inverses(); P->sys_valid = true;
     return 0;
 }
-static int fit_stage_windows(RingFit &f) {
+static bool fit_stage_wanted(const RingFit &f) { return f.ctx->opt("solve_staged", 1) != 0 && f.P->nr_b < 32768 && f.P->nc_b < 32768; }
+static int fit_stage_plan(RingFit &f) {
     cnmfe_ctx *ctx = f.ctx; Patch *P = f.P;
-    if (!(f.packed && ctx->opt("solve_staged", 1) != 0 && P->nr_b < 32768 && P->nc_b < 32768)) return 0;
     static thread_local std::vector<int> nmeta, lmeta;
-    const int64_t tot = plan::stage_windows(f.K, fit_nbox, f.L.lst_k, P->nr_b, P->nc_b, f.reach.p_radius, nmeta, lmeta);
+    const int64_t tot = f.stage_tot = plan::stage_windows(f.K, fit_nbox, f.L.lst_k, P->nr_b, P->nc_b, f.reach.p_radius, nmeta, lmeta);
+    f.stage_planned = true;
     if (tot < 0) return 0;
-    f.stage_ok = true;
     RET(to_dev(ctx, ctx->stg[0], nmeta)); RET(to_dev(ctx, ctx->stg[1], lmeta));
     RET(ctx->stg[2].ensure((size_t)std::max<int64_t>(1, tot) * sizeof(double)));
     RET(ctx->stg[3].ensure((size_t)std::max<int64_t>(1, tot) * sizeof(float)));
+    return 0;
+}
+static int fit_stage_windows(RingFit &f) {
+    cnmfe_ctx *ctx = f.ctx;
+    if (!(f.packed && fit_stage_wanted(f))) return 0;
+    if (!f.stage_planned) RET(fit_stage_plan(f));
+    if (f.stage_tot < 0) return 0;
+    f.stage_ok = true;
     int *dErrW = nullptr;
     RET(ctx_errflag(ctx, &dErrW));
     LAUNCH(ctx, "bg_neuron_windows", k_nwin_build, dim3((unsigned)f.K), dim3(256), 0, ctx->stg[0].as<int>(), f.g, (int)f.K, f.dArow.as<int>(), f.dAcol.as<int>(), f.dAval.as<float>(),
            f.dLp->as<int>(), f.dSlot->as<short>(), f.dUt.as<double>(), ctx->stg[2].as<double>(), ctx->stg[3].as<float>(), dErrW);
+    return 0;
+}
+static int fit_slot_table(RingFit &f) {
+    const size_t bytes = (size_t)f.nblk * std::max(1, (int)f.K) * sizeof(short);
+    RET(f.dSlot->ensure(bytes));
+    CK(hipMemsetAsync(f.dSlot->p, 0xff, bytes, f.ctx->st()));
+    LAUNCH(f.ctx, "bg_slot_table", k_slot_build, dim3((unsigned)f.nblk), dim3(64), 0, f.dLp->as<int>(), f.dLk.as<int>(), (int)f.K, f.dSlot->as<short>());
+    return 0;
+}
+static int fit_side_setup(RingFit &f) {
+    cnmfe_ctx *ctx = f.ctx; Patch *P = f.P;
+    LAUNCH(ctx, "bg_trace_subsum", k_trace_subsum, dim3(f.K), dim3(256), 0, f.dCc.as<float>(), f.ldc, f.g.Tp, f.g.kstride, f.dCsum.as<double>());
+    if (f.win_i8) RET(fit_trace_gram(f));
+    RET(fit_upload_csr(f));
+    f.ht.mark("A csr");
+    RET(fit_active_b0(f));
+    f.ht.mark("ind_active + b0");
+    RET(fit_slot_table(f));
+    if (f.incr && pack_wanted(ctx, f.nt) && P->sys_valid && P->sys.cap >= sys_bytes_of(P->d, f.nt) && (int64_t)f.nblk * std::max(1, f.K) < (int64_t)1 << 31 &&
+        (int64_t)f.L.lst_k.size() * BLKPX < (int64_t)1 << 31 && fit_stage_wanted(f)) RET(fit_stage_plan(f));
+    f.setup_done = true;
     return 0;
 }
 static int fit_corrections(RingFit &f, const float *C, int c_order) {
@@ -875,7 +991,7 @@
         return 0;
     }
     if (!f.proj_queued) RET(fit_queue_projection(f));
-    RET(to_dev(ctx, *f.dSlot, f.L.slot_of));
+    if (!f.setup_done) RET(fit_slot_table(f));
     if (f.keep_pt) RET(P->pt_tab.ensure(std::max<size_t>(1, f.L.lst_k.size()) * BLKPX * sizeof(double)));
     LAUNCH(ctx, "bg_win_fix", k_win_fix, dim3((unsigned)f.L.blall.size(), WIN_NLB / WF_S), dim3(256), 0, g, K, f.dArow.as<int>(), f.dAcol.as<int>(), f.dAval.as<float>(), f.dLp->as<int>(),
            f.dSlot->as<short>(), f.dBl.as<int>(), f.nsg, f.dUt.as<double>(), f.ut_stride, f.dGb.as<double>(), f.gb_stride, f.keep_pt ? P->pt_tab.as<double>() : nullptr,
@@ -886,6 +1002,7 @@
         P->pt_valid = true;
     }
     const int csplit = f.npairs >= 8192 ? 1 : f.npairs >= 4096 ? 2 : 4;
+    if (!f.packed) RET(fit_need_tables(f));
     if (!f.packed)
         LAUNCH(ctx, "bg_cov_correct", k_cov_correct, dim3((unsigned)f.npairs, (unsigned)csplit), dim3(256), 0, P->cov_base.as<double>(), ctx->cov.as<double>(), f.dPairs.as<int4>(),
                f.dNeed.as<unsigned short>(), g, K, f.dArow.as<int>(), f.dAcol.as<int>(), f.dAval.as<float>(), f.dLp->as<int>(), f.dSlot->as<short>(), f.dUt.as<double>());
@@ -974,12 +1091,14 @@
     }
     RET(fit_geometry(f, with_projection));
     fit_lists(f);
-    if (f.incr && f.has_a && !f.build_base) RET(fit_queue_projection(f));
+    if (f.incr && f.has_a && !f.build_base) RET(fit_queue_projection(f, fit_side_mode(f)));
     f.ht.mark("projection queued");
-    RET(fit_upload_csr(f));
-    f.ht.mark("A csr");
-    RET(fit_active_b0(f));
-    f.ht.mark("ind_active + b0");
+    if (!f.setup_done) {
+        RET(fit_upload_csr(f));
+        f.ht.mark("A csr");
+        RET(fit_active_b0(f));
+        f.ht.mark("ind_active + b0");
+    }
     RET(fit_pair_tables(f));
     if (!f.incr || f.build_base) RET(fit_base_table(f));
     if (f.nt < 1 || f.nt > 8) return fail(CNMFE_EUNSUPPORTED, "fit_ring_model: %d ring neighbours (<= %d supported)", P->p, PMAX_RING);
diff --git a/cnmf_e_amd/csrc/common.hpp b/cnmf_e_amd/csrc/common.hpp
--- a/cnmf_e_amd/csrc/common.hpp
+++ b/cnmf_e_amd/csrc/common.hpp
@@ -12,6 +12,7 @@
 #include <map>
 #include <algorithm>
 #include "../../include/cnmfe.h"
+#include "ring_plan.hpp"
 
 namespace cnmfe {
 
@@ -160,6 +161,13 @@
     bool base_valid = false, derived = false;
     int base_kstride = 0;
     DevBuf cov_base_alt, rowsum_base_alt; bool base_alt_valid = false; int base_alt_kstride = 0;
+    struct RingTabs {
+        bool keyed = false, built = false;
+        int geo[8] = {0, 0, 0, 0, 0, 0, 0, 0}; std::vector<int32_t> dr, dc;
+        int npairs = 0, nwork = 0;
+        std::vector<plan::Pair> pairs; std::vector<int> pair_of; plan::Tables tabs;
+        DevBuf dPairs, dPairOf, dWork, dNeed, dTcnt, dTl;
+    } rt;
     DevBuf sys, sys_alt; bool sys_valid = false, sys_alt_valid = false;
     DevBuf kinv, kinv_lam, kinv_list; bool kinv_valid = false, kinv_lam_valid = false; int kinv_fits = 0;
     void drop_inverses() { kinv_valid = false; kinv_lam_valid = false; kinv_fits = 0; }
@@ -248,6 +256,7 @@
     cnmfe::PinArena pin;
     int64_t spatial_nnz = -1;
     hipStream_t copy_stream = nullptr;
+    hipStream_t side_stream = nullptr; hipEvent_t ev_side_fork = nullptr, ev_side_join = nullptr;
     hipEvent_t ev_bound_ready = nullptr, ev_copy_done = nullptr; bool copy_pending = false;
     int64_t copy_gen = 0; std::vector<std::pair<int64_t, hipEvent_t>> copy_gens; std::vector<hipEvent_t> copy_ev_pool;
     int copy_batch_mark();
@@ -436,6 +445,7 @@
 int ring_stats_get(cnmfe_ctx *ctx, Patch *P, int *pmax, bool *first);
 int center_traces(cnmfe_ctx *ctx, const float *C, int64_t ldc, int32_t K, int64_t T, DevBuf &Cc, DevBuf &Cmean);
 int upload_centered(cnmfe_ctx *ctx, DevBuf &stage, const float *C, int32_t K, int64_t T, int order, DevBuf &Cc, DevBuf &Cmean, int64_t *ldc_out);
+int ctx_side_stream(cnmfe_ctx *ctx);
 int ctx_errflag(cnmfe_ctx *ctx, int **dflag);
 int ctx_check_errflag(cnmfe_ctx *ctx);
 }
```
